# simzero/cudaParticlesFoam

Hardware: AMD Instinct MI355X
Metric: Mparticle-steps/s (higher is better)
Workload: dtype f64

## Files before the change

cudaparticlesfoam_amd/csrc/cpf_api.cpp:

```cpp
#include <hip/hip_runtime.h>

#include <algorithm>
#include <cmath>
#include <cstring>
#include <condition_variable>
#include <mutex>
#include <string>
#include <thread>
#include <utility>
#include <vector>

#include "cpf.h"
#include "cpf_device.h"
#include "cpf_internal.h"
#include "cpf_walk.h"

struct cpf_context {
    int device = 0;
    hipStream_t ownStream = nullptr, stream = nullptr;
    mutable std::string err;
    bool haveMesh = false, haveU = false;
    cpf::HostTables host;
    int32_t* d_cellOff = nullptr;
    double4* d_planes = nullptr;
    int32_t* d_nbr = nullptr;
    int32_t *d_groupOff = nullptr, *d_groupNbr = nullptr;
    bool zFold = true;
    double4* d_U = nullptr;
    double* d_U3 = nullptr;
    double* d_boxRec = nullptr;
    bool boxRecords = true;
    double4* d_cellRec = nullptr;
    unsigned long long* d_occupied = nullptr;
    hipEvent_t evFieldFlag = nullptr;
    bool fieldFlagPending = false;
    unsigned long long* h_occupied = nullptr;
    int64_t nSecondRecords = 0;
    float* d_cellBox = nullptr;
    int32_t* d_curveRank = nullptr;
    int sortMethod = 2;
    int sortCurve = -1;
    int32_t* d_binOff = nullptr;
    int32_t* d_binCells = nullptr;
    size_t meshBytes = 0;
    int64_t cap = 0, n = 0;
    double *x = nullptr, *y = nullptr, *z = nullptr, *vel = nullptr;
    int32_t* cell = nullptr;
    int64_t* gid = nullptr;
    double *x2 = nullptr, *y2 = nullptr, *z2 = nullptr;
    int32_t* cell2 = nullptr;
    int64_t* gid2 = nullptr;
    bool located = false;
    void* scratch = nullptr;
    size_t scratchBytes = 0;
    unsigned long long* d_counters = nullptr;
    uint32_t seed = 1591593751u;
    uint32_t stepCounter = 0;
    int sortInterval = 50;
    uint32_t lastSortStep = 0;
    bool stats = false;
    int stepVariant = -1;
    bool vtuBinary = false;
    bool mixedRecords = true;
    double nonplanarTol = cpf::kNonPlanarTolDefault;
    bool splitNonplanar = true;
    cpf_mesh_quality quality{};
    int64_t nParent = 0;
    std::vector<int32_t> first;
    int32_t* d_parentOf = nullptr;
    double* d_Uparent = nullptr;
    cpf::StreamState streamState;
    int64_t lastStepN = -1;
    int lastStepCycles = 1;
    bool zSettled = false;
    bool lastStepZSettled = false;
    double* d_tetPos = nullptr; int32_t* d_tets = nullptr; double* d_vertVel = nullptr;
    int64_t nTetVerts = 0, nTets = 0; int tetsPerCell = 0; bool haveVertVel = false;
    double* d_vertCone = nullptr;
    double* d_vertApex = nullptr;
    bool vertexFast = true;
    std::string vertConeWhy;
    std::thread writer;
    bool writerLive = false;
    int writerStatus = CPF_OK;
    void* snapDev = nullptr; void* snapHost = nullptr;
    size_t snapBytes = 0;
    hipStream_t ioStream = nullptr;
    hipEvent_t evSnap = nullptr, evCopied = nullptr;
    double frameKE = 0.0;
    std::mutex keMutex; std::condition_variable keCv; bool keReady = false;
    int timingStride = 1;
    uint64_t timingLaunch = 0;
    bool timing = false;
    std::vector<std::pair<hipEvent_t, hipEvent_t>> events;
    std::vector<hipEvent_t> eventPool;
};

namespace {

std::string g_createError = "";
std::mutex g_mutex;

struct WriterRegistry {
    std::vector<cpf_context*> live;
    ~WriterRegistry();
} g_writers;

int fail(const cpf_context* ctx, int code, const std::string& msg) {
    if (ctx) ctx->err = msg;
    else { std::lock_guard<std::mutex> lk(g_mutex); g_createError = msg; }
    return code;
}

#define CPF_HIP(ctx, call)                                                                              \
    do {                                                                                                \
        hipError_t e__ = (call);                                                                        \
        if (e__ != hipSuccess)                                                                          \
            return fail(ctx, CPF_ERR_HIP, std::string(#call) + ": " + hipGetErrorString(e__));          \
    } while (0)

#define CPF_REQUIRE(ctx, cond, code, msg) \
    do { if (!(cond)) return fail(ctx, code, msg); } while (0)

template <typename T>
void freeDev(T*& p) { if (p) { (void)hipFree(p); p = nullptr; } }

cpf::MeshView meshView(const cpf_context* c) {
    cpf::MeshView m;
    m.cellOff = c->d_cellOff; m.planes = c->d_planes; m.nbr = c->d_nbr; m.U = c->d_U;
    m.groupOff = c->d_groupOff; m.groupNbr = c->d_groupNbr;
    m.cellRec = c->d_cellRec;
    m.boxRec = c->boxRecords ? reinterpret_cast<const double4*>(c->d_boxRec) : nullptr;
    m.nCells = (int32_t)c->host.nCells;
    m.allHex = (c->host.minCellFaces == 6 && c->host.maxCellFaces == 6 && c->host.nGroups() == 0) ? 1 : 0;
    m.zPairLast = c->host.zPairLast ? 1 : 0;
    m.zThin = (c->host.zThin && c->zFold) ? 1 : 0;
    m.zSide0 = c->host.zSide0 ? 1 : 0;
    m.mixed = (c->d_cellRec && !m.allHex) ? (c->host.nBigCells > 0 ? 2 : 1) : 0;
    return m;
}
cpf::GridView gridView(const cpf_context* c) {
    cpf::GridView g;
    for (int k = 0; k < 3; ++k) {
        g.origin[k] = c->host.origin[k]; g.invBin[k] = c->host.invBin[k];
        g.lo[k] = c->host.lo[k]; g.hi[k] = c->host.hi[k]; g.dims[k] = c->host.dims[k];
    }
    g.binOff = c->d_binOff; g.binCells = c->d_binCells;
    return g;
}

int ensureScratch(cpf_context* ctx, size_t bytes) {
    if (bytes <= ctx->scratchBytes) return CPF_OK;
    CPF_HIP(ctx, hipStreamSynchronize(ctx->stream));
    freeDev(ctx->scratch);
    ctx->scratchBytes = 0;
    CPF_HIP(ctx, hipMalloc(&ctx->scratch, bytes));
    ctx->scratchBytes = bytes;
    return CPF_OK;
}

int sortEndBit(const cpf_context* ctx) {
    int bits = 1;
    while (((int64_t)1 << bits) < ctx->host.nCells + 2) ++bits;
    return std::min(bits + ctx->host.subBits[0] + ctx->host.subBits[1] + ctx->host.subBits[2], 32);
}

void freeMesh(cpf_context* c) {
    freeDev(c->d_cellOff); freeDev(c->d_planes); freeDev(c->d_nbr); freeDev(c->d_groupOff); freeDev(c->d_groupNbr); freeDev(c->d_U); freeDev(c->d_U3); freeDev(c->d_cellRec); freeDev(c->d_boxRec); freeDev(c->d_cellBox); freeDev(c->d_curveRank);
    freeDev(c->d_binOff); freeDev(c->d_binCells);
    c->haveMesh = c->haveU = false; c->meshBytes = 0;
    c->nSecondRecords = 0;
    freeDev(c->d_parentOf); freeDev(c->d_Uparent);
    c->first.clear(); c->nParent = 0; c->quality = cpf_mesh_quality{};
    freeDev(c->d_tetPos); freeDev(c->d_tets); freeDev(c->d_vertVel);
    c->haveVertVel = false; c->nTets = c->nTetVerts = 0; c->tetsPerCell = 0;
}
void freeCloud(cpf_context* c) {
    freeDev(c->x); freeDev(c->y); freeDev(c->z); freeDev(c->vel); freeDev(c->cell); freeDev(c->gid);
    freeDev(c->x2); freeDev(c->y2); freeDev(c->z2); freeDev(c->cell2); freeDev(c->gid2);
    c->cap = c->n = 0; c->located = false; c->zSettled = false;
}

cpf_mesh_quality toQuality(const cpf::MeshQuality& q, int64_t nDerived) {
    cpf_mesh_quality r{};
    r.maxNonPlanarity = q.maxEta; r.worstFace = q.worstFace;
    r.maxNonConvexity = q.maxXi; r.worstCell = q.worstCell;
    r.nCells = q.nCells; r.nFlaggedCells = q.nFlagged; r.nBadCells = q.nBad; r.nDerivedCells = nDerived;
    r.tol = q.tol;
    return r;
}

template <typename Label>
int setMeshImpl(cpf_context* ctx, const double* points, int64_t nPoints, const Label* faceOffsets,
                const Label* faceVerts, int64_t nFaces, const Label* owner, const Label* neighbour,
                int64_t nInternal, int64_t nCells) {
    CPF_REQUIRE(ctx, ctx, CPF_ERR_ARG, "null context");
    CPF_REQUIRE(ctx, points && faceOffsets && faceVerts && owner && (neighbour || nInternal == 0), CPF_ERR_ARG,
                "cpf_set_mesh: null array");
    cpf::MeshQuality q;
    std::string why = cpf::measure_mesh<Label>(points, nPoints, faceOffsets, faceVerts, nFaces, owner, neighbour, nInternal,
                                               nCells, ctx->nonplanarTol, q);
    if (!why.empty()) return fail(ctx, CPF_ERR_MESH, "cpf_set_mesh: " + why);
    bool derive = ctx->splitNonplanar && q.decompose();
    cpf::DerivedMesh dm;
    cpf::HostTables t;
    if (derive) {
        why = cpf::derive_mesh<Label>(points, nPoints, faceOffsets, faceVerts, nFaces, owner, neighbour, nInternal, nCells, q, dm);
        if (why.empty())
            why = cpf::build_tables<int64_t>(dm.points.data(), dm.nPoints, dm.faceOff.data(), dm.faceVerts.data(), dm.nFaces,
                                             dm.owner.data(), dm.neighbour.data(), dm.nInternal, dm.nCells, t);
        for (int64_t c = 0; c < nCells && why.empty() && derive; ++c)
            if (dm.first[(size_t)c + 1] - dm.first[(size_t)c] == 1) {
                const int32_t d = dm.first[(size_t)c];
                if (t.cellOff[(size_t)d + 1] - t.cellOff[(size_t)d] > q.cellOff[(size_t)c + 1] - q.cellOff[(size_t)c]) derive = false;
            }
    }
    if (!derive) {
        why = cpf::build_tables<Label>(points, nPoints, faceOffsets, faceVerts, nFaces, owner, neighbour, nInternal, nCells, t);
    }
    if (!why.empty()) return fail(ctx, CPF_ERR_MESH, "cpf_set_mesh: " + why);
    CPF_HIP(ctx, hipSetDevice(ctx->device));
    CPF_HIP(ctx, hipStreamSynchronize(ctx->stream));
    freeMesh(ctx);
    ctx->streamState.flatField = false;
    ctx->host = std::move(t);
    ctx->nParent = nCells;
    ctx->quality = toQuality(q, ctx->host.nCells);
    nCells = ctx->host.nCells;
    const cpf::HostTables& h = ctx->host;
    auto up = [&](auto*& dptr, const void* src, size_t bytes) -> hipError_t {
        hipError_t e = hipMalloc((void**)&dptr, std::max<size_t>(bytes, 16));
        if (e != hipSuccess) return e;
        ctx->meshBytes += bytes;
        return hipMemcpy(dptr, src, bytes, hipMemcpyHostToDevice);
    };
    CPF_HIP(ctx, up(ctx->d_cellOff, h.cellOff.data(), h.cellOff.size() * 4));
    CPF_HIP(ctx, up(ctx->d_planes, h.planes.data(), h.planes.size() * 8));
    CPF_HIP(ctx, up(ctx->d_nbr, h.nbr.data(), h.nbr.size() * 4));
    CPF_HIP(ctx, up(ctx->d_groupOff, h.groupOff.data(), h.groupOff.size() * 4));
    CPF_HIP(ctx, up(ctx->d_groupNbr, h.groupNbr.data(), h.groupNbr.size() * 4));
    CPF_HIP(ctx, up(ctx->d_binOff, h.binOff.data(), h.binOff.size() * 4));
    CPF_HIP(ctx, up(ctx->d_binCells, h.binCells.data(), h.binCells.size() * 4));
    CPF_HIP(ctx, up(ctx->d_cellBox, h.cellBox.data(), h.cellBox.size() * 4));
    CPF_HIP(ctx, up(ctx->d_curveRank, h.curveRank.data(), h.curveRank.size() * 4));
    if (derive) {
        ctx->first = std::move(dm.first);
        CPF_HIP(ctx, up(ctx->d_parentOf, dm.parent.data(), dm.parent.size() * 4));
        CPF_HIP(ctx, hipMalloc((void**)&ctx->d_Uparent, (size_t)ctx->nParent * 3 * sizeof(double)));
        ctx->meshBytes += (size_t)ctx->nParent * 24;
    }
    CPF_HIP(ctx, hipMalloc((void**)&ctx->d_U, (size_t)nCells * sizeof(double4)));
    CPF_HIP(ctx, hipMalloc((void**)&ctx->d_U3, (size_t)nCells * 3 * sizeof(double)));
    CPF_HIP(ctx, hipMemset(ctx->d_U, 0, (size_t)nCells * sizeof(double4)));
    if (ctx->host.minCellFaces == 6 && ctx->host.maxCellFaces == 6 && ctx->host.nGroups() == 0) {
        CPF_HIP(ctx, hipMalloc((void**)&ctx->d_cellRec, (size_t)nCells * 8 * sizeof(double4)));
        CPF_HIP(ctx, cpf::launch_build_cell_records(ctx->stream, ctx->d_planes, ctx->d_nbr, ctx->d_U, ctx->d_cellRec, nCells));
        CPF_HIP(ctx, hipStreamSynchronize(ctx->stream));
        ctx->meshBytes += (size_t)nCells * 256;
        if (!h.boxRec.empty()) CPF_HIP(ctx, up(ctx->d_boxRec, h.boxRec.data(), h.boxRec.size() * 8));
    } else if (ctx->host.nHugeCells * 4 <= nCells && ctx->mixedRecords) {
        std::vector<int32_t> recB((size_t)nCells, -1);
        int64_t nSecond = 0;
        for (int64_t c = 0; c < nCells; ++c) {
            const int nf = ctx->host.cellOff[(size_t)c + 1] - ctx->host.cellOff[(size_t)c];
            if (nf > 6 && nf <= 12) recB[(size_t)c] = (int32_t)(nCells + nSecond++);
        }
        CPF_REQUIRE(ctx, nCells + nSecond < ((int64_t)1 << 31), CPF_ERR_MESH, "cpf_set_mesh: too many cell records");
        int32_t* d_recB = nullptr;
        hipError_t e = hipSuccess;
        if (nSecond > 0) e = up(d_recB, recB.data(), recB.size() * 4);
        if (e == hipSuccess) e = hipMalloc((void**)&ctx->d_cellRec, (size_t)(nCells + nSecond) * 8 * sizeof(double4));
        if (e == hipSuccess) e = cpf::launch_build_cell_records_mixed(ctx->stream, ctx->d_cellOff, ctx->d_planes, ctx->d_nbr, ctx->d_U, d_recB,
                                                                      ctx->d_cellRec, nCells);
        if (e == hipSuccess) e = hipStreamSynchronize(ctx->stream);
        freeDev(d_recB);
        CPF_HIP(ctx, e);
        ctx->nSecondRecords = nSecond;
        ctx->meshBytes += (size_t)(nCells + nSecond) * 256;
        if (!h.boxRec.empty() && nSecond == 0) CPF_HIP(ctx, up(ctx->d_boxRec, h.boxRec.data(), h.boxRec.size() * 8));
    }
    ctx->meshBytes += (size_t)nCells * (sizeof(double4) + 24);
    ctx->haveMesh = true;
    ctx->located = false;
    ctx->zSettled = false;
    if (ctx->h_occupied) ctx->h_occupied[0] = ctx->h_occupied[1] = 0;
    return CPF_OK;
}

}

namespace {
WriterRegistry::~WriterRegistry() {
    for (cpf_context* c : live)
        if (c->writerLive && c->writer.joinable()) { c->writer.join(); c->writerLive = false; }
}
}

namespace cpf {
bool vtu_binary(const cpf_context* ctx) { return ctx && ctx->vtuBinary; }
bool context_derived(const cpf_context* ctx) { return ctx && ctx->d_parentOf != nullptr; }
void* context_stream(const cpf_context* ctx) { return (void*)ctx->stream; }
int context_device(const cpf_context* ctx) { return ctx->device; }
bool context_timing(const cpf_context* ctx) { return ctx->timing; }
int64_t context_cells(const cpf_context* ctx) { return ctx->haveMesh ? ctx->host.nCells : 0; }
bool context_step_settled_z(const cpf_context* ctx) { return ctx->lastStepZSettled; }
}

namespace {
std::string tetFanDefect(const double* pos, const int32_t* tets, int64_t nCells, int tetsPerCell) {
    auto P = [&](int32_t v, int k) { return pos[3 * (int64_t)v + k]; };
    const double fourPi = 12.566370614359172;
    std::vector<uint64_t> edges;
    for (int64_t c = 0; c < nCells; ++c) {
        const int32_t* t0 = tets + 4 * c * tetsPerCell;
        const int32_t apex = t0[0];
        double omega = 0.0;
        int sign = 0;
        for (int k = 0; k < tetsPerCell; ++k) {
            const int32_t* ix = t0 + 4 * k;
            if (ix[0] != apex) return "cell " + std::to_string(c) + ": its tets do not share their first vertex";
            double e[3][3], len[3];
            for (int j = 0; j < 3; ++j) {
                for (int q = 0; q < 3; ++q) e[j][q] = P(ix[j + 1], q) - P(apex, q);
                len[j] = std::sqrt(e[j][0] * e[j][0] + e[j][1] * e[j][1] + e[j][2] * e[j][2]);
            }
            const double det = e[0][0] * (e[1][1] * e[2][2] - e[1][2] * e[2][1]) - e[0][1] * (e[1][0] * e[2][2] - e[1][2] * e[2][0]) +
                               e[0][2] * (e[1][0] * e[2][1] - e[1][1] * e[2][0]);
            const double scale = len[0] * len[1] * len[2];
            if (!(std::fabs(det) * 1e5 > scale)) return "cell " + std::to_string(c) + ": a flat (or badly conditioned) tet";
            const int sg = det > 0 ? 1 : -1;
            if (sign == 0) sign = sg;
            else if (sg != sign) return "cell " + std::to_string(c) + ": tets of both orientations";
            auto dot = [&](int i, int j) { return e[i][0] * e[j][0] + e[i][1] * e[j][1] + e[i][2] * e[j][2]; };
            omega += 2.0 * std::atan2(std::fabs(det), scale + dot(0, 1) * len[2] + dot(0, 2) * len[1] + dot(1, 2) * len[0]);
        }
        if (std::fabs(omega - fourPi) > 1e-6) return "cell " + std::to_string(c) + ": the tets' solid angles at the apex do not add up to 4 pi";
        edges.clear();
        for (int k = 0; k < tetsPerCell; ++k) {
            const int32_t* ix = t0 + 4 * k;
            for (int j = 0; j < 3; ++j) edges.push_back(((uint64_t)(uint32_t)ix[1 + j] << 32) | (uint32_t)ix[1 + (j + 1) % 3]);
        }
        std::sort(edges.begin(), edges.end());
        for (size_t i = 0; i < edges.size(); ++i) {
            const uint64_t rev = (edges[i] << 32) | (edges[i] >> 32);
            if ((i > 0 && edges[i] == edges[i - 1]) || !std::binary_search(edges.begin(), edges.end(), rev))
                return "cell " + std::to_string(c) + ": the tets' base triangles do not form a closed surface";
        }
    }
    return "";
}

hipError_t layOutField(cpf_context* ctx, const double* dU3, int64_t nCells) {
    const bool ask = ctx->host.zSide0 && ctx->d_occupied && ctx->h_occupied;
    ctx->streamState.flatField = false;
    ctx->fieldFlagPending = false;
    hipError_t e = hipSuccess;
    if (ask) e = hipMemsetAsync(ctx->d_occupied + 2, 0, 8, ctx->stream);
    if (e == hipSuccess) e = cpf::launch_u3_to_u4(ctx->stream, dU3, ctx->d_U, nCells, ask ? ctx->d_occupied + 2 : nullptr);
    if (e == hipSuccess && ctx->d_cellRec) e = cpf::launch_update_record_velocity(ctx->stream, ctx->d_U, ctx->d_cellRec, ctx->d_boxRec, nCells);
    if (e == hipSuccess && ask) {
        e = hipMemcpyAsync(ctx->h_occupied + 2, ctx->d_occupied + 2, 8, hipMemcpyDeviceToHost, ctx->stream);
        if (e == hipSuccess) e = hipEventRecord(ctx->evFieldFlag, ctx->stream);
        ctx->fieldFlagPending = e == hipSuccess;
    }
    return e;
}
std::string resolveSubCells(const cpf_context* ctx, int64_t n, const double* xyz, const int32_t* cell, std::vector<int32_t>& out) {
    const cpf::HostTables& h = ctx->host;
    out.resize((size_t)n);
    for (int64_t i = 0; i < n; ++i) {
        const int32_t c = cell[i];
        if (c < 0) { out[(size_t)i] = c; continue; }
        if (c >= ctx->nParent) return "cell[" + std::to_string(i) + "] = " + std::to_string(c) + " is not a cell of the mesh";
        const double px = xyz[3 * i], py = xyz[3 * i + 1], pz = xyz[3 * i + 2];
        int32_t pick = ctx->first[(size_t)c];
        double pickWorst = HUGE_VAL;
        for (int32_t d = ctx->first[(size_t)c]; d < ctx->first[(size_t)c + 1]; ++d) {
            double worst = -HUGE_VAL;
            for (int32_t s = h.cellOff[(size_t)d]; s < h.cellOff[(size_t)d + 1]; ++s) {
                const double* pl = &h.planes[4 * (size_t)s];
                worst = std::max(worst, std::fma(-pl[2], pz, std::fma(-pl[1], py, std::fma(-pl[0], px, pl[3]))));
            }
            if (worst < cpf::kTol) { pick = d; break; }
            if (worst < pickWorst) { pickWorst = worst; pick = d; }
        }
        out[(size_t)i] = pick;
    }
    return std::string();
}
void fieldFlagArrived(cpf_context* ctx) {
    if (!ctx->fieldFlagPending) return;
    ctx->streamState.flatField = ctx->h_occupied[2] == 0;
    ctx->fieldFlagPending = false;
}
void pollFieldFlag(cpf_context* ctx) {
    if (ctx->fieldFlagPending && hipEventQuery(ctx->evFieldFlag) == hipSuccess) fieldFlagArrived(ctx);
}
}

extern "C" {

int cpf_abi_version(void) { return CPF_ABI_VERSION; }

int cpf_create(int device, cpf_context** out) {
    if (!out) return fail(nullptr, CPF_ERR_ARG, "cpf_create: out is null");
    *out = nullptr;
    int count = 0;
    hipError_t e = hipGetDeviceCount(&count);
    if (e != hipSuccess || count <= 0)
        return fail(nullptr, CPF_ERR_HIP,
                    std::string("cpf_create: no HIP device available (") + hipGetErrorString(e) + ")");
    if (device < 0 || device >= count) return fail(nullptr, CPF_ERR_ARG, "cpf_create: device index out of range");
    e = hipSetDevice(device);
    if (e != hipSuccess) return fail(nullptr, CPF_ERR_HIP, std::string("hipSetDevice: ") + hipGetErrorString(e));
    cpf_context* ctx = new (std::nothrow) cpf_context();
    if (!ctx) return fail(nullptr, CPF_ERR_NOMEM, "cpf_create: out of host memory");
    ctx->device = device;
    e = hipStreamCreateWithFlags(&ctx->ownStream, hipStreamNonBlocking);
    if (e == hipSuccess) e = hipMalloc((void**)&ctx->d_counters, (cpf::kCounterSlots * 4 + 4) * sizeof(unsigned long long));
    if (e == hipSuccess) e = hipMemset(ctx->d_counters, 0, (cpf::kCounterSlots * 4 + 4) * sizeof(unsigned long long));
    if (e == hipSuccess) e = hipMalloc((void**)&ctx->d_occupied, 32);
    if (e == hipSuccess) e = hipHostMalloc((void**)&ctx->h_occupied, 32, hipHostMallocDefault);
    if (e == hipSuccess) { ctx->h_occupied[0] = ctx->h_occupied[1] = 0; ctx->h_occupied[2] = 1; ctx->streamState.occupiedHost = ctx->h_occupied; }
    if (e == hipSuccess) e = hipEventCreateWithFlags(&ctx->evFieldFlag, hipEventDisableTiming);
    if (e == hipSuccess) e = hipMalloc((void**)&ctx->streamState.d_grab, cpf::kStreamGrabBytes);
    if (e == hipSuccess) e = hipMemset(ctx->streamState.d_grab, 0, cpf::kStreamGrabBytes);
    if (e == hipSuccess) {
        int cus = 0;
        e = hipDeviceGetAttribute(&cus, hipDeviceAttributeMultiprocessorCount, device);
        if (e == hipSuccess && cus > 0) ctx->streamState.numCU = cus;
    }
    if (e == hipSuccess) {
        ctx->streamState.hitSpillWaves = 32 * ctx->streamState.numCU;
        e = hipMalloc((void**)&ctx->streamState.d_hitSpill,
                      (size_t)ctx->streamState.hitSpillWaves * cpf::kStreamHitSpillDoubles * sizeof(double));
    }
    if (e != hipSuccess) {
        std::string m = std::string("cpf_create: ") + hipGetErrorString(e);
        if (ctx->ownStream) (void)hipStreamDestroy(ctx->ownStream);
        delete ctx;
        return fail(nullptr, CPF_ERR_HIP, m);
    }
    ctx->stream = ctx->ownStream;
    *out = ctx;
    return CPF_OK;
}

int cpf_destroy(cpf_context* ctx) {
    if (!ctx) return CPF_OK;
    (void)cpf_write_vtu_wait(ctx);
    (void)hipSetDevice(ctx->device);
    (void)hipStreamSynchronize(ctx->stream);
    freeMesh(ctx); freeCloud(ctx);
    freeDev(ctx->scratch); freeDev(ctx->d_counters); freeDev(ctx->streamState.d_grab); freeDev(ctx->streamState.d_hitSpill);
    freeDev(ctx->d_occupied);
    if (ctx->evFieldFlag) { (void)hipEventDestroy(ctx->evFieldFlag); ctx->evFieldFlag = nullptr; }
    if (ctx->h_occupied) { (void)hipHostFree(ctx->h_occupied); ctx->h_occupied = nullptr; ctx->streamState.occupiedHost = nullptr; }
    freeDev(ctx->d_tetPos); freeDev(ctx->d_tets); freeDev(ctx->d_vertVel); freeDev(ctx->d_vertCone); freeDev(ctx->d_vertApex);
    freeDev(ctx->snapDev);
    if (ctx->snapHost) { (void)hipHostFree(ctx->snapHost); ctx->snapHost = nullptr; }
    if (ctx->evSnap) (void)hipEventDestroy(ctx->evSnap);
    if (ctx->evCopied) (void)hipEventDestroy(ctx->evCopied);
    if (ctx->ioStream) (void)hipStreamDestroy(ctx->ioStream);
    for (auto& p : ctx->events) { (void)hipEventDestroy(p.first); (void)hipEventDestroy(p.second); }
    for (auto& ev : ctx->eventPool) (void)hipEventDestroy(ev);
    if (ctx->ownStream) (void)hipStreamDestroy(ctx->ownStream);
    delete ctx;
    return CPF_OK;
}

const char* cpf_last_error(const cpf_context* ctx) {
    if (ctx) return ctx->err.c_str();
    std::lock_guard<std::mutex> lk(g_mutex);
    return g_createError.c_str();
}

int cpf_set_stream(cpf_context* ctx, void* hip_stream) {
    CPF_REQUIRE(ctx, ctx, CPF_ERR_ARG, "null context");
    CPF_HIP(ctx, hipStreamSynchronize(ctx->stream));
    fieldFlagArrived(ctx);
    ctx->stream = (hipStream_t)hip_stream;
    return CPF_OK;
}

int cpf_use_own_stream(cpf_context* ctx) {
    CPF_REQUIRE(ctx, ctx, CPF_ERR_ARG, "null context");
    CPF_HIP(ctx, hipStreamSynchronize(ctx->stream));
    fieldFlagArrived(ctx);
    ctx->stream = ctx->ownStream;
    return CPF_OK;
}

int cpf_synchronize(cpf_context* ctx) {
    CPF_REQUIRE(ctx, ctx, CPF_ERR_ARG, "null context");
    CPF_HIP(ctx, hipStreamSynchronize(ctx->stream));
    return CPF_OK;
}

int cpf_set_mesh(cpf_context* ctx, const double* points, int64_t nPoints, const int32_t* faceOffsets,
                 const int32_t* faceVerts, int64_t nFaces, const int32_t* owner, const int32_t* neighbour,
                 int64_t nInternal, int64_t nCells) {
    return setMeshImpl<int32_t>(ctx, points, nPoints, faceOffsets, faceVerts, nFaces, owner, neighbour, nInternal,
                                nCells);
}
int cpf_set_mesh_l64(cpf_context* ctx, const double* points, int64_t nPoints, const int64_t* faceOffsets,
                     const int64_t* faceVerts, int64_t nFaces, const int64_t* owner, const int64_t* neighbour,
                     int64_t nInternal, int64_t nCells) {
    return setMeshImpl<int64_t>(ctx, points, nPoints, faceOffsets, faceVerts, nFaces, owner, neighbour, nInternal,
                                nCells);
}

int cpf_build_mesh_tables_host(const double* points, int64_t nPoints, const int32_t* faceOffsets, const int32_t* faceVerts,
                               int64_t nFaces, const int32_t* owner, const int32_t* neighbour, int64_t nInternal, int64_t nCells,
                               int64_t* nSlots, int64_t* nGroups, int64_t* nMembers, int32_t* cellOff, double* planes,
                               int32_t* nbr, int32_t* groupOff, int32_t* groupNbr) {
    if (!points || !faceOffsets || !faceVerts || !owner || (!neighbour && nInternal != 0)) return CPF_ERR_ARG;
    cpf::HostTables t;
    try {
        const std::string why = cpf::build_tables<int32_t>(points, nPoints, faceOffsets, faceVerts, nFaces, owner, neighbour, nInternal, nCells, t);
        if (!why.empty()) return CPF_ERR_MESH;
    } catch (const std::bad_alloc&) {
        return CPF_ERR_NOMEM;
    }
    const int64_t g = t.nGroups(), mem = t.groupOff[(size_t)g];
    if (nSlots) *nSlots = t.nSlots;
    if (nGroups) *nGroups = g;
    if (nMembers) *nMembers = mem;
    if (cellOff) std::memcpy(cellOff, t.cellOff.data(), t.cellOff.size() * 4);
    if (planes) std::memcpy(planes, t.planes.data(), t.planes.size() * 8);
    if (nbr) std::memcpy(nbr, t.nbr.data(), t.nbr.size() * 4);
    if (groupOff) std::memcpy(groupOff, t.groupOff.data(), (size_t)(g + 1) * 4);
    if (groupNbr) std::memcpy(groupNbr, t.groupNbr.data(), (size_t)mem * 4);
    return CPF_OK;
}

int cpf_mesh_flags_host(const double* points, int64_t nPoints, const int32_t* faceOffsets, const int32_t* faceVerts,
                        int64_t nFaces, const int32_t* owner, const int32_t* neighbour, int64_t nInternal, int64_t nCells,
                        int32_t* allHex, int32_t* zLayered, int32_t* zThin, int32_t* mixed) {
    if (!points || !faceOffsets || !faceVerts || !owner || (!neighbour && nInternal != 0)) return CPF_ERR_ARG;
    cpf::HostTables t;
    try {
        const std::string why = cpf::build_tables<int32_t>(points, nPoints, faceOffsets, faceVerts, nFaces, owner, neighbour, nInternal, nCells, t);
        if (!why.empty()) return CPF_ERR_MESH;
    } catch (const std::bad_alloc&) {
        return CPF_ERR_NOMEM;
    }
    const bool hex = t.minCellFaces == 6 && t.maxCellFaces == 6 && t.nGroups() == 0;
    if (allHex) *allHex = hex ? 1 : 0;
    if (zLayered) *zLayered = t.zPairLast ? 1 : 0;
    if (zThin) *zThin = t.zThin ? 1 : 0;
    if (mixed) *mixed = hex ? 0 : (t.nHugeCells * 4 <= nCells ? (t.nBigCells > 0 ? 2 : 1) : 0);
    return CPF_OK;
}

int cpf_mesh_box_records_host(const double* points, int64_t nPoints, const int32_t* faceOffsets, const int32_t* faceVerts,
                              int64_t nFaces, const int32_t* owner, const int32_t* neighbour, int64_t nInternal, int64_t nCells,
                              int32_t* isBox, double* boxRec) {
    if (!points || !faceOffsets || !faceVerts || !owner || (!neighbour && nInternal != 0)) return CPF_ERR_ARG;
    cpf::HostTables t;
    try {
        const std::string why = cpf::build_tables<int32_t>(points, nPoints, faceOffsets, faceVerts, nFaces, owner, neighbour, nInternal, nCells, t);
        if (!why.empty()) return CPF_ERR_MESH;
    } catch (const std::bad_alloc&) {
        return CPF_ERR_NOMEM;
    }
    if (isBox) *isBox = t.boxRec.empty() ? 0 : 1;
    if (boxRec && !t.boxRec.empty()) std::memcpy(boxRec, t.boxRec.data(), t.boxRec.size() * 8);
    return CPF_OK;
}

int cpf_mesh_quality_host(const double* points, int64_t nPoints, const int32_t* faceOffsets, const int32_t* faceVerts,
                          int64_t nFaces, const int32_t* owner, const int32_t* neighbour, int64_t nInternal, int64_t nCells,
                          double tol, int split, cpf_mesh_quality* out) {
    if (!points || !faceOffsets || !faceVerts || !owner || (!neighbour && nInternal != 0) || !out || !(tol > 0.0)) return CPF_ERR_ARG;
    try {
        cpf::MeshQuality q;
        if (!cpf::measure_mesh<int32_t>(points, nPoints, faceOffsets, faceVerts, nFaces, owner, neighbour, nInternal, nCells, tol, q).empty())
            return CPF_ERR_MESH;
        int64_t nDerived = nCells;
        if (split && q.decompose()) {
            cpf::DerivedMesh dm;
            if (!cpf::derive_mesh<int32_t>(points, nPoints, faceOffsets, faceVerts, nFaces, owner, neighbour, nInternal, nCells, q, dm).empty())
                return CPF_ERR_MESH;
            nDerived = dm.nCells;
        }
        *out = toQuality(q, nDerived);
    } catch (const std::bad_alloc&) {
        return CPF_ERR_NOMEM;
    }
    return CPF_OK;
}

int cpf_build_derived_mesh_host(const double* points, int64_t nPoints, const int32_t* faceOffsets, const int32_t* faceVerts,
                                int64_t nFaces, const int32_t* owner, const int32_t* neighbour, int64_t nInternal, int64_t nCells,
                                double tol, int64_t sizes[5], double* pointsOut, int32_t* faceOffOut, int32_t* faceVertsOut,
                                int32_t* ownerOut, int32_t* neighbourOut, int32_t* first) {
    if (!points || !faceOffsets || !faceVerts || !owner || (!neighbour && nInternal != 0) || !sizes || !(tol > 0.0)) return CPF_ERR_ARG;
    try {
        cpf::MeshQuality q;
        if (!cpf::measure_mesh<int32_t>(points, nPoints, faceOffsets, faceVerts, nFaces, owner, neighbour, nInternal, nCells, tol, q).empty())
            return CPF_ERR_MESH;
        cpf::DerivedMesh dm;
        if (!cpf::derive_mesh<int32_t>(points, nPoints, faceOffsets, faceVerts, nFaces, owner, neighbour, nInternal, nCells, q, dm).empty())
            return CPF_ERR_MESH;
        if (dm.faceVerts.size() > (size_t)INT32_MAX) return CPF_ERR_MESH;
        sizes[0] = dm.nPoints; sizes[1] = dm.nFaces; sizes[2] = (int64_t)dm.faceVerts.size(); sizes[3] = dm.nInternal; sizes[4] = dm.nCells;
        auto narrow = [](const std::vector<int64_t>& v, int32_t* o) { if (o) for (size_t i = 0; i < v.size(); ++i) o[i] = (int32_t)v[i]; };
        if (pointsOut) std::memcpy(pointsOut, dm.points.data(), dm.points.size() * 8);
        narrow(dm.faceOff, faceOffOut); narrow(dm.faceVerts, faceVertsOut); narrow(dm.owner, ownerOut); narrow(dm.neighbour, neighbourOut);
        if (first) std::memcpy(first, dm.first.data(), dm.first.size() * 4);
    } catch (const std::bad_alloc&) {
        return CPF_ERR_NOMEM;
    }
    return CPF_OK;
}

int cpf_get_mesh_quality(const cpf_context* ctx, cpf_mesh_quality* out) {
    CPF_REQUIRE(ctx, ctx && out, CPF_ERR_ARG, "null argument");
    CPF_REQUIRE(ctx, ctx->haveMesh, CPF_ERR_STATE, "cpf_get_mesh_quality: call cpf_set_mesh first");
    *out = ctx->quality;
    return CPF_OK;
}

int cpf_cells_to_parent_dev(cpf_context* ctx, const int32_t* in, int32_t* out, int64_t n) {
    CPF_REQUIRE(ctx, ctx, CPF_ERR_ARG, "null context");
    CPF_REQUIRE(ctx, ctx->haveMesh, CPF_ERR_STATE, "cpf_cells_to_parent_dev: call cpf_set_mesh first");
    CPF_REQUIRE(ctx, n >= 0 && (n == 0 || (in && out)), CPF_ERR_ARG, "cpf_cells_to_parent_dev: bad arguments");
    CPF_HIP(ctx, hipSetDevice(ctx->device));
    if (ctx->d_parentOf) CPF_HIP(ctx, cpf::launch_cells_to_parent(ctx->stream, in, out, ctx->d_parentOf, n, ctx->host.nCells));
    else if (n > 0 && in != out) CPF_HIP(ctx, hipMemcpyAsync(out, in, (size_t)n * 4, hipMemcpyDeviceToDevice, ctx->stream));
    return CPF_OK;
}

int cpf_mesh_info(const cpf_context* ctx, int64_t* nCells, int64_t* nSlots, int64_t* deviceBytes) {
    CPF_REQUIRE(ctx, ctx, CPF_ERR_ARG, "null context");
    CPF_REQUIRE(ctx, ctx->haveMesh, CPF_ERR_STATE, "cpf_mesh_info: no mesh set");
    if (nCells) *nCells = ctx->host.nCells;
    if (nSlots) *nSlots = ctx->host.nSlots;
    if (deviceBytes) *deviceBytes = (int64_t)ctx->meshBytes;
    return CPF_OK;
}

int cpf_get_mesh_tables(const cpf_context* ctx, int32_t* cellOff, double* planes, int32_t* nbr) {
    CPF_REQUIRE(ctx, ctx, CPF_ERR_ARG, "null context");
    CPF_REQUIRE(ctx, ctx->haveMesh, CPF_ERR_STATE, "cpf_get_mesh_tables: no mesh set");
    const cpf::HostTables& h = ctx->host;
    if (cellOff) std::memcpy(cellOff, h.cellOff.data(), h.cellOff.size() * 4);
    if (planes) std::memcpy(planes, h.planes.data(), h.planes.size() * 8);
    if (nbr) std::memcpy(nbr, h.nbr.data(), h.nbr.size() * 4);
    return CPF_OK;
}

int cpf_get_mesh_groups(const cpf_context* ctx, int64_t* nGroups, int64_t* nMembers, int32_t* groupOff, int32_t* groupNbr) {
    CPF_REQUIRE(ctx, ctx, CPF_ERR_ARG, "null context");
    CPF_REQUIRE(ctx, ctx->haveMesh, CPF_ERR_STATE, "cpf_get_mesh_groups: no mesh set");
    const cpf::HostTables& h = ctx->host;
    const int64_t g = h.nGroups();
    if (nGroups) *nGroups = g;
    if (nMembers) *nMembers = h.groupOff[(size_t)g];
    if (groupOff) std::memcpy(groupOff, h.groupOff.data(), (size_t)(g + 1) * 4);
    if (groupNbr) std::memcpy(groupNbr, h.groupNbr.data(), (size_t)h.groupOff[(size_t)g] * 4);
    return CPF_OK;
}

int cpf_get_mesh_flags(const cpf_context* ctx, int32_t* allHex, int32_t* zLayered, int32_t* zThin, int32_t* mixed) {
    CPF_REQUIRE(ctx, ctx, CPF_ERR_ARG, "null context");
    CPF_REQUIRE(ctx, ctx->haveMesh, CPF_ERR_STATE, "cpf_get_mesh_flags: no mesh set");
    const cpf::MeshView m = meshView(ctx);
    if (allHex) *allHex = m.allHex;
    if (zLayered) *zLayered = m.zPairLast;
    if (zThin) *zThin = m.zThin;
    if (mixed) *mixed = m.mixed;
    return CPF_OK;
}

int cpf_set_velocity(cpf_context* ctx, const double* U, int64_t nCells) {
    CPF_REQUIRE(ctx, ctx, CPF_ERR_ARG, "null context");
    CPF_REQUIRE(ctx, ctx->haveMesh, CPF_ERR_STATE, "cpf_set_velocity: call cpf_set_mesh first");
    CPF_REQUIRE(ctx, U && nCells == ctx->nParent, CPF_ERR_ARG, "cpf_set_velocity: U is null or nCells differs from the mesh");
    CPF_HIP(ctx, hipSetDevice(ctx->device));
    if (ctx->d_parentOf) {
        CPF_HIP(ctx, hipMemcpyAsync(ctx->d_Uparent, U, (size_t)nCells * 24, hipMemcpyHostToDevice, ctx->stream));
        CPF_HIP(ctx, cpf::launch_gather_parent_u3(ctx->stream, ctx->d_Uparent, ctx->d_parentOf, ctx->d_U3, ctx->host.nCells));
    } else {
        CPF_HIP(ctx, hipMemcpyAsync(ctx->d_U3, U, (size_t)nCells * 24, hipMemcpyHostToDevice, ctx->stream));
    }
    CPF_HIP(ctx, layOutField(ctx, ctx->d_U3, ctx->host.nCells));
    CPF_HIP(ctx, hipStreamSynchronize(ctx->stream));
    fieldFlagArrived(ctx);
    ctx->haveU = true;
    return CPF_OK;
}

int cpf_set_velocity_dev(cpf_context* ctx, const double* dU, int64_t nCells) {
    CPF_REQUIRE(ctx, ctx, CPF_ERR_ARG, "null context");
    CPF_REQUIRE(ctx, ctx->haveMesh, CPF_ERR_STATE, "cpf_set_velocity_dev: call cpf_set_mesh first");
    CPF_REQUIRE(ctx, dU && nCells == ctx->nParent, CPF_ERR_ARG, "cpf_set_velocity_dev: bad arguments");
    CPF_HIP(ctx, hipSetDevice(ctx->device));
    if (ctx->d_parentOf) {
        CPF_HIP(ctx, cpf::launch_gather_parent_u3(ctx->stream, dU, ctx->d_parentOf, ctx->d_U3, ctx->host.nCells));
        dU = ctx->d_U3;
    }
    CPF_HIP(ctx, layOutField(ctx, dU, ctx->host.nCells));
    ctx->haveU = true;
    return CPF_OK;
}

int cpf_alloc_particles(cpf_context* ctx, int64_t capacity) {
    CPF_REQUIRE(ctx, ctx, CPF_ERR_ARG, "null context");
    CPF_REQUIRE(ctx, capacity > 0 && capacity < ((int64_t)1 << 31), CPF_ERR_ARG, "cpf_alloc_particles: capacity must be in (0, 2^31)");
    CPF_HIP(ctx, hipSetDevice(ctx->device));
    CPF_HIP(ctx, hipStreamSynchronize(ctx->stream));
    freeCloud(ctx);
    const size_t c = (size_t)capacity;
    CPF_HIP(ctx, hipMalloc((void**)&ctx->x, c * 8));
    CPF_HIP(ctx, hipMalloc((void**)&ctx->y, c * 8));
    CPF_HIP(ctx, hipMalloc((void**)&ctx->z, c * 8));
    CPF_HIP(ctx, hipMalloc((void**)&ctx->vel, c * 24));
    CPF_HIP(ctx, hipMalloc((void**)&ctx->cell, c * 4));
    CPF_HIP(ctx, hipMalloc((void**)&ctx->gid, c * 8));
    CPF_HIP(ctx, hipMemsetAsync(ctx->vel, 0, c * 24, ctx->stream));
    CPF_HIP(ctx, hipMemsetAsync(ctx->cell, 0xFF, c * 4, ctx->stream));
    ctx->cap = capacity;
    return CPF_OK;
}

int cpf_seed_box(cpf_context* ctx, int64_t n, const double lower[3], const double upper[3], int order) {
    CPF_REQUIRE(ctx, ctx, CPF_ERR_ARG, "null context");
    CPF_REQUIRE(ctx, lower && upper && n > 0, CPF_ERR_ARG, "cpf_seed_box: bad arguments");
    if (ctx->cap < n) { int r = cpf_alloc_particles(ctx, n); if (r) return r; }
    CPF_HIP(ctx, hipSetDevice(ctx->device));
    CPF_HIP(ctx, cpf::launch_seed_box(ctx->stream, ctx->x, ctx->y, ctx->z, 0, n, lower, upper, order));
    CPF_HIP(ctx, cpf::launch_iota64(ctx->stream, ctx->gid, n, 0));
    CPF_HIP(ctx, hipMemsetAsync(ctx->cell, 0xFF, (size_t)n * 4, ctx->stream));
    ctx->n = n; ctx->located = false; ctx->zSettled = false;
    return CPF_OK;
}

int cpf_set_particles(cpf_context* ctx, int64_t n, const double* xyz, const int32_t* cell) {
    CPF_REQUIRE(ctx, ctx, CPF_ERR_ARG, "null context");
    CPF_REQUIRE(ctx, xyz && n > 0, CPF_ERR_ARG, "cpf_set_particles: bad arguments");
    if (ctx->cap < n) { int r = cpf_alloc_particles(ctx, n); if (r) return r; }
    CPF_HIP(ctx, hipSetDevice(ctx->device));
    ctx->zSettled = false;
    int r = ensureScratch(ctx, (size_t)n * 24);
    if (r) return r;
    CPF_HIP(ctx, hipMemcpyAsync(ctx->scratch, xyz, (size_t)n * 24, hipMemcpyHostToDevice, ctx->stream));
    CPF_HIP(ctx, cpf::launch_unpack_xyz(ctx->stream, (const double*)ctx->scratch, ctx->x, ctx->y, ctx->z, n));
    CPF_HIP(ctx, cpf::launch_iota64(ctx->stream, ctx->gid, n, 0));
    std::vector<int32_t> sub;
    if (cell && ctx->d_parentOf) {
        std::string why = resolveSubCells(ctx, n, xyz, cell, sub);
        if (!why.empty()) { (void)hipStreamSynchronize(ctx->stream); return fail(ctx, CPF_ERR_ARG, "cpf_set_particles: " + why); }
        cell = sub.data();
    }
    if (cell) CPF_HIP(ctx, hipMemcpyAsync(ctx->cell, cell, (size_t)n * 4, hipMemcpyHostToDevice, ctx->stream));
    else CPF_HIP(ctx, hipMemsetAsync(ctx->cell, 0xFF, (size_t)n * 4, ctx->stream));
    CPF_HIP(ctx, hipStreamSynchronize(ctx->stream));
    ctx->n = n; ctx->located = cell != nullptr;
    return CPF_OK;
}

int cpf_locate_initial_dev(cpf_context* ctx, const double* x, const double* y, const double* z, int32_t* cell,
                           int64_t n) {
    CPF_REQUIRE(ctx, ctx, CPF_ERR_ARG, "null context");
    CPF_REQUIRE(ctx, ctx->haveMesh, CPF_ERR_STATE, "cpf_locate_initial: call cpf_set_mesh first");
    CPF_REQUIRE(ctx, n >= 0 && (n == 0 || (x && y && z && cell)), CPF_ERR_ARG, "cpf_locate_initial: null array");
    CPF_HIP(ctx, hipSetDevice(ctx->device));
    CPF_HIP(ctx, cpf::launch_locate_initial(ctx->stream, x, y, z, cell, n, meshView(ctx), gridView(ctx)));
    return CPF_OK;
}

int cpf_locate_initial(cpf_context* ctx, int64_t* nOutside) {
    CPF_REQUIRE(ctx, ctx, CPF_ERR_ARG, "null context");
    CPF_REQUIRE(ctx, ctx->n > 0, CPF_ERR_STATE, "cpf_locate_initial: no particles (seed or set them first)");
    ctx->zSettled = false;
    int r = cpf_locate_initial_dev(ctx, ctx->x, ctx->y, ctx->z, ctx->cell, ctx->n);
    if (r) return r;
    ctx->located = true;
    if (nOutside) {
        unsigned long long* cnt = ctx->d_counters + cpf::kCounterSlots * 4;
        CPF_HIP(ctx, hipMemsetAsync(cnt, 0, 8, ctx->stream));
        CPF_HIP(ctx, cpf::launch_count_negative(ctx->stream, ctx->cell, ctx->n, cnt));
        unsigned long long h = 0;
        CPF_HIP(ctx, hipMemcpyAsync(&h, cnt, 8, hipMemcpyDeviceToHost, ctx->stream));
        CPF_HIP(ctx, hipStreamSynchronize(ctx->stream));
        *nOutside = (int64_t)h;
    }
    return CPF_OK;
}

static cpf::VertexField vertexField(const cpf_context* ctx) {
    return {ctx->d_tetPos, ctx->d_tets, ctx->d_vertVel, ctx->tetsPerCell, ctx->vertexFast ? ctx->d_vertCone : nullptr,
            reinterpret_cast<const double4*>(ctx->d_vertApex)};
}

#ifndef CPF_TIMING_EVENT_FLAGS
#define CPF_TIMING_EVENT_FLAGS hipEventReleaseToDevice
#endif

int cpf_step_dev(cpf_context* ctx, double* x, double* y, double* z, int32_t* cell, const int64_t* gid, double* vel,
                 int64_t n, double dt, double D, uint32_t step0, int nCycles, unsigned flags) {
    CPF_REQUIRE(ctx, ctx, CPF_ERR_ARG, "null context");
    CPF_REQUIRE(ctx, ctx->haveMesh, CPF_ERR_STATE, "cpf_step: call cpf_set_mesh first");
    CPF_REQUIRE(ctx, ctx->haveU, CPF_ERR_STATE, "cpf_step: call cpf_set_velocity first");
    CPF_REQUIRE(ctx, n >= 0 && nCycles >= 0, CPF_ERR_ARG, "cpf_step: negative count");
    CPF_REQUIRE(ctx, n == 0 || (x && y && z && cell), CPF_ERR_ARG, "cpf_step: null particle array");
    CPF_REQUIRE(ctx, std::isfinite(dt) && std::isfinite(D) && D >= 0.0, CPF_ERR_ARG, "cpf_step: dt/D not finite or D < 0");
    CPF_REQUIRE(ctx, !(flags & CPF_STEP_STORE_VEL) || vel, CPF_ERR_ARG, "cpf_step: CPF_STEP_STORE_VEL needs a vel array");
    CPF_HIP(ctx, hipSetDevice(ctx->device));
    const bool vertexU = (flags & CPF_STEP_VERTEX_VELOCITY) != 0;
    CPF_REQUIRE(ctx, !vertexU || (ctx->haveVertVel && ctx->nTets == (int64_t)ctx->tetsPerCell * ctx->host.nCells), CPF_ERR_STATE,
                "cpf_step: CPF_STEP_VERTEX_VELOCITY needs cpf_set_tets and cpf_set_vertex_velocity for the current mesh");
    const cpf::MeshView m = meshView(ctx);
    const cpf::VertexField vf = vertexField(ctx);
    const bool fuse = (flags & CPF_STEP_FUSE_CYCLES) != 0;
    pollFieldFlag(ctx);
    bool settled = (flags & CPF_STEP_Z_SETTLED) != 0;
    ctx->lastStepZSettled = false;
    const int nLaunch = fuse ? 1 : nCycles;
    const int cycPerLaunch = fuse ? nCycles : 1;
    for (int c = 0; c < nLaunch; ++c) {
        const cpf::StepPlan plan = cpf::plan_step(m, ctx->streamState, ctx->stepVariant, vertexU ? &vf : nullptr, n, cycPerLaunch, D,
                                                  flags, ctx->stats);
        hipEvent_t e0 = nullptr, e1 = nullptr;
        const bool timed = ctx->timing && (ctx->timingLaunch++ % (uint64_t)ctx->timingStride) == 0;
        const bool stamped = timed && n > 0 && plan.stamped();
        if (timed) {
            auto take = [&](hipEvent_t& ev) -> hipError_t {
                if (!ctx->eventPool.empty()) { ev = ctx->eventPool.back(); ctx->eventPool.pop_back(); return hipSuccess; }
                return hipEventCreateWithFlags(&ev, CPF_TIMING_EVENT_FLAGS);
            };
            CPF_HIP(ctx, take(e0)); CPF_HIP(ctx, take(e1));
            if (!stamped) CPF_HIP(ctx, hipEventRecord(e0, ctx->stream));
        }
        ctx->lastStepN = n; ctx->lastStepCycles = cycPerLaunch;
        const hipError_t le = cpf::launch_step(plan, ctx->stream, x, y, z, cell, gid, vel, n, dt, D, step0 + (uint32_t)c, cycPerLaunch,
                                               ctx->seed, m, ctx->stats ? ctx->d_counters : nullptr, vertexU ? &vf : nullptr,
                                               ctx->streamState, settled, stamped ? e0 : nullptr, stamped ? e1 : nullptr);
        if (le != hipSuccess) {
            if (e0) ctx->eventPool.push_back(e0);
            if (e1) ctx->eventPool.push_back(e1);
        }
        CPF_HIP(ctx, le);
        if (n > 0 && cycPerLaunch > 0) settled = plan.flat();
        if (timed) {
            if (!stamped) CPF_HIP(ctx, hipEventRecord(e1, ctx->stream));
            ctx->events.emplace_back(e0, e1);
        }
    }
    ctx->lastStepZSettled = settled;
    return CPF_OK;
}

int cpf_step(cpf_context* ctx, double dt, double D, int nCycles, unsigned flags) {
    CPF_REQUIRE(ctx, ctx, CPF_ERR_ARG, "null context");
    CPF_REQUIRE(ctx, ctx->n > 0, CPF_ERR_STATE, "cpf_step: no particles");
    CPF_REQUIRE(ctx, ctx->located, CPF_ERR_STATE, "cpf_step: particles have no cells yet (call cpf_locate_initial)");
    if ((flags & CPF_STEP_STORE_VEL) && ctx->vel) {
        CPF_HIP(ctx, hipSetDevice(ctx->device));
        CPF_HIP(ctx, hipMemsetAsync(ctx->vel, 0, (size_t)ctx->n * 24, ctx->stream));
    }
    const bool settled = ctx->zSettled;
    ctx->zSettled = false;
    int r = cpf_step_dev(ctx, ctx->x, ctx->y, ctx->z, ctx->cell, ctx->gid, ctx->vel, ctx->n, dt, D, ctx->stepCounter,
                         nCycles, (flags & ~CPF_STEP_Z_SETTLED) | (settled ? CPF_STEP_Z_SETTLED : 0u));
    if (r != CPF_OK) return r;
    ctx->zSettled = ctx->lastStepZSettled;
    if (!(dt == 0.0 && D == 0.0)) ctx->stepCounter += (uint32_t)nCycles;
    if (ctx->sortInterval > 0 && ctx->stepCounter - ctx->lastSortStep >= (uint32_t)ctx->sortInterval) {
        r = cpf_sort_by_cell(ctx);
        ctx->lastSortStep = ctx->stepCounter;
    }
    return r;
}

int cpf_seed_box_dev(cpf_context* ctx, double* x, double* y, double* z, int64_t first, int64_t n,
                     const double lower[3], const double upper[3], int order) {
    CPF_REQUIRE(ctx, ctx, CPF_ERR_ARG, "null context");
    CPF_REQUIRE(ctx, n >= 0 && first >= 0 && lower && upper && (n == 0 || (x && y && z)), CPF_ERR_ARG, "cpf_seed_box_dev: bad arguments");
    CPF_HIP(ctx, hipSetDevice(ctx->device));
    CPF_HIP(ctx, cpf::launch_seed_box(ctx->stream, x, y, z, first, n, lower, upper, order));
    return CPF_OK;
}

namespace {
int sortImpl(cpf_context* ctx, double* x, double* y, double* z, int32_t* cell, int64_t* gid, int64_t n, double* ox, double* oy,
             double* oz, int32_t* ocell, int64_t* ogid, double* vel3) {
    CPF_REQUIRE(ctx, ctx->haveMesh, CPF_ERR_STATE, "cpf_sort_by_cell: call cpf_set_mesh first");
    CPF_REQUIRE(ctx, n >= 0 && n < ((int64_t)1 << 31) && (n == 0 || (x && y && z && cell)), CPF_ERR_ARG, "cpf_sort_by_cell: bad arguments");
    CPF_REQUIRE(ctx, ctx->host.nCells < ((int64_t)1 << 26) - 2, CPF_ERR_STATE, "cpf_sort_by_cell: more than 2^26 cells");
    CPF_HIP(ctx, hipSetDevice(ctx->device));
    const int endBit = sortEndBit(ctx);
    const bool census = ctx->streamState.densityLookup != 0 && ctx->d_occupied && ctx->h_occupied;
    const bool curve = ctx->d_curveRank != nullptr && (ctx->sortCurve == 1 || (ctx->sortCurve < 0 && n < 8 * ctx->host.nCells));
    int r = ensureScratch(ctx, cpf::sort_scratch_bytes(n, endBit));
    if (r) return r;
    CPF_HIP(ctx, cpf::sort_by_cell(ctx->stream, x, y, z, cell, gid, vel3, n, endBit, ctx->d_cellBox, ctx->host.subBits,
                                   ctx->host.subOrder, ctx->scratch, ctx->scratchBytes, ox, oy, oz, ocell, ogid, census ? ctx->d_occupied : nullptr,
                                   curve ? ctx->d_curveRank : nullptr, ctx->sortMethod));
    if (census)
        CPF_HIP(ctx, hipMemcpyAsync(ctx->h_occupied, ctx->d_occupied, 16, hipMemcpyDeviceToHost, ctx->stream));
    return CPF_OK;
}
}

int cpf_sort_by_cell_dev(cpf_context* ctx, double* x, double* y, double* z, int32_t* cell, int64_t* gid, int64_t n) {
    CPF_REQUIRE(ctx, ctx, CPF_ERR_ARG, "null context");
    if (n <= 1) return CPF_OK;
    return sortImpl(ctx, x, y, z, cell, gid, n, nullptr, nullptr, nullptr, nullptr, nullptr, nullptr);
}

int cpf_sort_by_cell_dev_to(cpf_context* ctx, const double* x, const double* y, const double* z, const int32_t* cell,
                            const int64_t* gid, double* ox, double* oy, double* oz, int32_t* ocell, int64_t* ogid, int64_t n) {
    CPF_REQUIRE(ctx, ctx, CPF_ERR_ARG, "null context");
    CPF_REQUIRE(ctx, n == 0 || (ox && oy && oz && ocell && (ogid || !gid)), CPF_ERR_ARG, "cpf_sort_by_cell_dev_to: null output array");
    CPF_REQUIRE(ctx, n == 0 || (ox != x && oy != y && oz != z && ocell != cell), CPF_ERR_ARG, "cpf_sort_by_cell_dev_to: outputs alias inputs");
    if (n <= 0) return CPF_OK;
    if (n == 1) {
        CPF_HIP(ctx, hipSetDevice(ctx->device));
        CPF_HIP(ctx, hipMemcpyAsync(ox, x, 8, hipMemcpyDeviceToDevice, ctx->stream));
        CPF_HIP(ctx, hipMemcpyAsync(oy, y, 8, hipMemcpyDeviceToDevice, ctx->stream));
        CPF_HIP(ctx, hipMemcpyAsync(oz, z, 8, hipMemcpyDeviceToDevice, ctx->stream));
        CPF_HIP(ctx, hipMemcpyAsync(ocell, cell, 4, hipMemcpyDeviceToDevice, ctx->stream));
        if (gid) CPF_HIP(ctx, hipMemcpyAsync(ogid, gid, 8, hipMemcpyDeviceToDevice, ctx->stream));
        return CPF_OK;
    }
    return sortImpl(ctx, const_cast<double*>(x), const_cast<double*>(y), const_cast<double*>(z), const_cast<int32_t*>(cell),
                    const_cast<int64_t*>(gid), n, ox, oy, oz, ocell, ogid, nullptr);
}

int cpf_sort_by_cell(cpf_context* ctx) {
    CPF_REQUIRE(ctx, ctx, CPF_ERR_ARG, "null context");
    CPF_REQUIRE(ctx, ctx->n > 0 && ctx->located, CPF_ERR_STATE, "cpf_sort_by_cell: no located particles");
    if (ctx->n <= 1) return CPF_OK;
    if (ctx->x2 == nullptr) {
        CPF_HIP(ctx, hipSetDevice(ctx->device));
        const size_t c = (size_t)ctx->cap;
        void* b[5] = {nullptr, nullptr, nullptr, nullptr, nullptr};
        const size_t bytes[5] = {c * 8, c * 8, c * 8, c * 4, c * 8};
        hipError_t e = hipSuccess;
        for (int k = 0; k < 5 && e == hipSuccess; ++k) e = hipMalloc(&b[k], bytes[k]);
        if (e == hipSuccess) e = hipMemsetAsync(b[3], 0xFF, bytes[3], ctx->stream);
        if (e != hipSuccess) {
            for (int k = 0; k < 5; ++k) if (b[k]) (void)hipFree(b[k]);
            CPF_HIP(ctx, e);
        }
        ctx->x2 = (double*)b[0]; ctx->y2 = (double*)b[1]; ctx->z2 = (double*)b[2];
        ctx->cell2 = (int32_t*)b[3]; ctx->gid2 = (int64_t*)b[4];
    }
    int r = sortImpl(ctx, ctx->x, ctx->y, ctx->z, ctx->cell, ctx->gid, ctx->n, ctx->x2, ctx->y2, ctx->z2, ctx->cell2, ctx->gid2,
                     ctx->vel);
    if (r) return r;
    std::swap(ctx->x, ctx->x2); std::swap(ctx->y, ctx->y2); std::swap(ctx->z, ctx->z2);
    std::swap(ctx->cell, ctx->cell2); std::swap(ctx->gid, ctx->gid2);
    return CPF_OK;
}

int cpf_num_particles(const cpf_context* ctx, int64_t* n) {
    CPF_REQUIRE(ctx, ctx && n, CPF_ERR_ARG, "null argument");
    *n = ctx->n;
    return CPF_OK;
}

int cpf_get_particles(cpf_context* ctx, double* xyzw, int32_t* cell, double* vel) {
    CPF_REQUIRE(ctx, ctx, CPF_ERR_ARG, "null context");
    CPF_REQUIRE(ctx, ctx->n > 0, CPF_ERR_STATE, "cpf_get_particles: no particles");
    CPF_HIP(ctx, hipSetDevice(ctx->device));
    const size_t n = (size_t)ctx->n;
    auto al = [](size_t b) { return (b + 255) & ~(size_t)255; };
    int r = ensureScratch(ctx, al(n * 32) + al(n * 4) + al(n * 32));
    if (r) return r;
    char* p = (char*)ctx->scratch;
    double* dX = (double*)p; p += al(n * 32);
    int32_t* dC = (int32_t*)p; p += al(n * 4);
    double* dV = (double*)p;
    CPF_HIP(ctx, cpf::launch_pack_by_gid(ctx->stream, ctx->x, ctx->y, ctx->z, ctx->cell, ctx->gid, ctx->vel,
                                         xyzw ? dX : nullptr, cell ? dC : nullptr, vel ? dV : nullptr, ctx->n));
    if (cell && ctx->d_parentOf) CPF_HIP(ctx, cpf::launch_cells_to_parent(ctx->stream, dC, dC, ctx->d_parentOf, ctx->n, ctx->host.nCells));
    if (xyzw) CPF_HIP(ctx, hipMemcpyAsync(xyzw, dX, n * 32, hipMemcpyDeviceToHost, ctx->stream));
    if (cell) CPF_HIP(ctx, hipMemcpyAsync(cell, dC, n * 4, hipMemcpyDeviceToHost, ctx->stream));
    if (vel) CPF_HIP(ctx, hipMemcpyAsync(vel, dV, n * 32, hipMemcpyDeviceToHost, ctx->stream));
    CPF_HIP(ctx, hipStreamSynchronize(ctx->stream));
    return CPF_OK;
}

int cpf_get_counters(cpf_context* ctx, int64_t out[4]) {
    CPF_REQUIRE(ctx, ctx && out, CPF_ERR_ARG, "null argument");
    CPF_HIP(ctx, hipSetDevice(ctx->device));
    std::vector<unsigned long long> h((size_t)cpf::kCounterSlots * 4);
    CPF_HIP(ctx, hipMemcpyAsync(h.data(), ctx->d_counters, h.size() * 8, hipMemcpyDeviceToHost, ctx->stream));
    CPF_HIP(ctx, hipStreamSynchronize(ctx->stream));
    for (int k = 0; k < 4; ++k) {
        unsigned long long sum = 0;
        for (int s = 0; s < cpf::kCounterSlots; ++s) sum += h[(size_t)s * 4 + k];
        out[k] = (int64_t)sum;
    }
    return CPF_OK;
}

int cpf_set_option(cpf_context* ctx, const char* key, double value) {
    CPF_REQUIRE(ctx, ctx && key, CPF_ERR_ARG, "null argument");
    const std::string k(key);
    if (k == "step_variant") {
        CPF_REQUIRE(ctx, value >= -1 && value <= 5 && value == (int)value, CPF_ERR_ARG, "step_variant must be -1..5");
#ifndef CPF_EXPERIMENTS
        CPF_REQUIRE(ctx, value != 1 && value != 2 && value != 5, CPF_ERR_ARG,
                    "step_variant 1, 2 and 5 are experiments (measured slower on every mesh) and not in this build: make EXPERIMENTS=1");
#endif
        ctx->stepVariant = (int)value;
        return CPF_OK;
    }
    if (k == "vertex_fast") {
        CPF_REQUIRE(ctx, value == 0 || value == 1, CPF_ERR_ARG, "vertex_fast must be 0 or 1");
        ctx->vertexFast = value != 0;
        return CPF_OK;
    }
    if (k == "z_fold") {
        CPF_REQUIRE(ctx, value == 0 || value == 1, CPF_ERR_ARG, "z_fold must be 0 or 1");
        ctx->zFold = value != 0;
        return CPF_OK;
    }
    if (k == "mixed_records") {
        CPF_REQUIRE(ctx, value == 0 || value == 1, CPF_ERR_ARG, "mixed_records must be 0 or 1");
        ctx->mixedRecords = value != 0;
        return CPF_OK;
    }
    if (k == "flat_walk") {
        CPF_REQUIRE(ctx, value == 0 || value == 1, CPF_ERR_ARG, "flat_walk must be 0 or 1");
        ctx->streamState.flat = (int)value;
        return CPF_OK;
    }
    if (k == "flat_z") {
        CPF_REQUIRE(ctx, value == 0 || value == 1, CPF_ERR_ARG, "flat_z must be 0 or 1");
        ctx->streamState.flatZ = (int)value;
        return CPF_OK;
    }
    if (k == "box_records") {
        CPF_REQUIRE(ctx, value == 0 || value == 1, CPF_ERR_ARG, "box_records must be 0 or 1");
        ctx->boxRecords = value != 0;
        return CPF_OK;
    }
    if (k == "stream_tiles_per_chunk") {
        CPF_REQUIRE(ctx, value >= 1 && value <= 1024 && value == (int)value, CPF_ERR_ARG, "stream_tiles_per_chunk must be 1..1024");
        ctx->streamState.tilesPerChunk = (int)value;
        return CPF_OK;
    }
    if (k == "sort_key_bits") {
        CPF_REQUIRE(ctx, ctx->haveMesh, CPF_ERR_STATE, "sort_key_bits: call cpf_set_mesh first");
        const int v = (int)value, nb[3] = {v / 100, (v / 10) % 10, v % 10};
        CPF_REQUIRE(ctx, value == v && v >= 0 && nb[0] <= 9 && nb[0] + nb[1] + nb[2] <= 12, CPF_ERR_ARG, "sort_key_bits: at most 12 bits");
        for (int a = 0; a < 3; ++a) {
            const float f = std::ldexp(1.0f, nb[a] - ctx->host.subBits[a]);
            for (size_t c = 0; c < ctx->host.cellBox.size() / 6; ++c) ctx->host.cellBox[6 * c + 3 + a] *= f;
            ctx->host.subBits[a] = nb[a];
        }
        CPF_HIP(ctx, hipSetDevice(ctx->device));
        CPF_HIP(ctx, hipMemcpyAsync(ctx->d_cellBox, ctx->host.cellBox.data(), ctx->host.cellBox.size() * 4, hipMemcpyHostToDevice, ctx->stream));
        CPF_HIP(ctx, hipStreamSynchronize(ctx->stream));
        return CPF_OK;
    }
    if (k == "stream_tail_fraction") {
        CPF_REQUIRE(ctx, value >= 0 && value <= 1, CPF_ERR_ARG, "stream_tail_fraction must be in [0, 1]");
        ctx->streamState.tailFraction = value;
        return CPF_OK;
    }
    if (k == "coop_max_cells") {
        CPF_REQUIRE(ctx, value >= 0 && value <= (1 << 24), CPF_ERR_ARG, "coop_max_cells must be in [0, 2^24]");
        ctx->streamState.coopMaxCells = (int)value;
        return CPF_OK;
    }
    if (k == "stream_lookup") {
        CPF_REQUIRE(ctx, value == -1 || (value >= 0 && value <= 6 && value == (int)value), CPF_ERR_ARG, "stream_lookup must be -1 (auto) or 0 ... 6");
        ctx->streamState.lookup = (int)value;
        return CPF_OK;
    }
    if (k == "stream_lookup_by_density") {
        CPF_REQUIRE(ctx, value == 0 || value == 1, CPF_ERR_ARG, "stream_lookup_by_density must be 0 or 1");
        ctx->streamState.densityLookup = (int)value;
        return CPF_OK;
    }
    if (k == "sort_method") {
        CPF_REQUIRE(ctx, value == 0 || value == 2, CPF_ERR_ARG, "sort_method must be 2 (this library's radix sort) or 0 (hipcub's)");
        ctx->sortMethod = (int)value;
        return CPF_OK;
    }
    if (k == "sort_curve") {
        CPF_REQUIRE(ctx, value == -1 || value == 0 || value == 1, CPF_ERR_ARG, "sort_curve must be -1 (by regime), 0 (cell id) or 1 (Morton rank)");
        ctx->sortCurve = (int)value;
        return CPF_OK;
    }
    if (k == "vtu_binary") {
        CPF_REQUIRE(ctx, value == 0 || value == 1, CPF_ERR_ARG, "vtu_binary must be 0 or 1");
        ctx->vtuBinary = value != 0;
        return CPF_OK;
    }
    if (k == "stream_debug") {
        ctx->streamState.debug = (int)value;
        return CPF_OK;
    }
    if (k == "stream_waves_per_cu") {
        CPF_REQUIRE(ctx, value >= 0 && value <= 32 && value == (int)value, CPF_ERR_ARG, "stream_waves_per_cu must be 0..32 (0 = auto)");
        ctx->streamState.wavesPerCU = (int)value;
        return CPF_OK;
    }
    if (k == "sort_interval") {
        CPF_REQUIRE(ctx, value >= 0 && value <= 1e9, CPF_ERR_ARG, "sort_interval must be >= 0 (0 = never)");
        ctx->sortInterval = (int)value;
        return CPF_OK;
    }
    if (k == "timing_stride") {
        CPF_REQUIRE(ctx, value >= 1 && value <= 1e6 && value == (int)value, CPF_ERR_ARG, "timing_stride must be an integer >= 1");
        ctx->timingStride = (int)value;
        return CPF_OK;
    }
    if (k == "stats") {
        ctx->stats = value != 0;
        return CPF_OK;
    }
    if (k == "nonplanar_tol") {
        CPF_REQUIRE(ctx, value > 0.0 && std::isfinite(value), CPF_ERR_ARG, "nonplanar_tol must be a positive number");
        ctx->nonplanarTol = value;
        return CPF_OK;
    }
    if (k == "split_nonplanar") {
        CPF_REQUIRE(ctx, value == 0 || value == 1, CPF_ERR_ARG, "split_nonplanar must be 0 or 1");
        ctx->splitNonplanar = value != 0;
        return CPF_OK;
    }
    return fail(ctx, CPF_ERR_ARG, "cpf_set_option: unknown key '" + k + "'");
}

}
namespace cpf {
void set_context_error(cpf_context* ctx, const char* message) {
    if (ctx) ctx->err = message ? message : "";
}
}
extern "C" {

int cpf_step_kernel_name(cpf_context* ctx, double D, unsigned flags, char* buf, size_t bufBytes) {
    CPF_REQUIRE(ctx, ctx && buf && bufBytes > 0, CPF_ERR_ARG, "null argument");
    CPF_REQUIRE(ctx, ctx->haveMesh, CPF_ERR_STATE, "cpf_step_kernel_name: call cpf_set_mesh first");
    const cpf::MeshView m = meshView(ctx);
    const cpf::VertexField vf = vertexField(ctx);
    pollFieldFlag(ctx);
    const bool vertexU = (flags & CPF_STEP_VERTEX_VELOCITY) != 0;
    const int64_t n = (vertexU ? ctx->lastStepN > 0 : ctx->lastStepN >= 0) ? ctx->lastStepN : ctx->n;
    const cpf::StepPlan p = cpf::plan_step(m, ctx->streamState, ctx->stepVariant, vertexU ? &vf : nullptr, n,
                                           (flags & CPF_STEP_FUSE_CYCLES) ? ctx->lastStepCycles : 1, D, flags, ctx->stats);
    const char* b[2] = {"false", "true"};
    char tmp[192];
    if (p.kernel == cpf::StepPlan::kStreamVertex)
        snprintf(tmp, sizeof tmp, "cpf::step_kernel_stream_vertex<%s, %s, %s, %s, %d> (cone locate)", b[p.brown], b[p.reflect],
                 b[p.storeVel], b[p.stats], p.lookup);
    else if (p.kernel == cpf::StepPlan::kVertex)
        snprintf(tmp, sizeof tmp, "cpf::step_kernel_vertex<%s, %s, %s> (%s)", b[p.brown], b[p.reflect], b[p.storeVel],
                 p.cone ? "cone locate" : (ctx->d_vertCone || ctx->vertConeWhy.empty() ? "all tets" : ("all tets: " + ctx->vertConeWhy).c_str()));
    else if (p.kernel == cpf::StepPlan::kAhead)
        snprintf(tmp, sizeof tmp, "cpf::step_kernel_ahead<%s, %s>", b[p.reflect], b[p.stats]);
    else if (p.kernel == cpf::StepPlan::kStream)
        snprintf(tmp, sizeof tmp, "cpf::step_kernel_stream<%s, %s, %s, %s, %d>", b[p.brown], b[p.reflect], b[p.storeVel], b[p.stats], p.lookup);
    else if (p.kernel == cpf::StepPlan::kCoop)
        snprintf(tmp, sizeof tmp, "cpf::step_kernel_coop<%s, %s, %s, %s>", b[p.brown], b[p.reflect], b[p.storeVel], b[p.stats]);
    else snprintf(tmp, sizeof tmp, "cpf::step_kernel<%d, %s, %s, %s>", (int)p.kernel, b[p.brown], b[p.reflect], b[p.storeVel]);
    snprintf(buf, bufBytes, "%s", tmp);
    return CPF_OK;
}

int cpf_set_seed(cpf_context* ctx, uint32_t seed) {
    CPF_REQUIRE(ctx, ctx, CPF_ERR_ARG, "null context");
    ctx->seed = seed;
    return CPF_OK;
}

int cpf_pack_leavers_dev(cpf_context* ctx, double* x, double* y, double* z, int32_t* cell, int64_t* gid, int64_t n,
                         const int32_t* cellLo_dev, int nRanks, int myRank, double* sendbuf, int64_t sendCapacity,
                         int64_t* counts_dev, int64_t* nStay_dev) {
    CPF_REQUIRE(ctx, ctx, CPF_ERR_ARG, "null context");
    CPF_REQUIRE(ctx, n >= 0 && n < ((int64_t)1 << 31) && nRanks >= 1 && nRanks <= CPF_MAX_RANKS && myRank >= 0 && myRank < nRanks,
                CPF_ERR_ARG, "cpf_pack_leavers_dev: bad sizes (1 .. CPF_MAX_RANKS ranks)");
    CPF_REQUIRE(ctx, cellLo_dev && counts_dev && nStay_dev && (sendbuf || sendCapacity == 0) && (n == 0 || (x && y && z && cell)),
                CPF_ERR_ARG, "cpf_pack_leavers_dev: null array");
    CPF_REQUIRE(ctx, !ctx->d_parentOf, CPF_ERR_MESH, "cpf_pack_leavers_dev: the mesh has cells decomposed into tets "
                "(cpf_get_mesh_quality): ownership ranges are parent ids, the cloud's cells derived ids");
    CPF_HIP(ctx, hipSetDevice(ctx->device));
    int r = ensureScratch(ctx, cpf::handoff_scratch_bytes(n, nRanks));
    if (r) return r;
    CPF_HIP(ctx, cpf::pack_leavers(ctx->stream, x, y, z, cell, gid, n, cellLo_dev, nRanks, myRank, sendbuf,
                                   sendCapacity, counts_dev, nStay_dev, ctx->scratch, ctx->scratchBytes));
    return CPF_OK;
}

int cpf_cell_histogram_dev(cpf_context* ctx, const int32_t* cell, int64_t n, double scale, double* weights_dev) {
    CPF_REQUIRE(ctx, ctx, CPF_ERR_ARG, "null context");
    CPF_REQUIRE(ctx, ctx->haveMesh, CPF_ERR_STATE, "cpf_cell_histogram_dev: call cpf_set_mesh first");
    CPF_REQUIRE(ctx, n >= 0 && weights_dev && (cell || n == 0), CPF_ERR_ARG, "cpf_cell_histogram_dev: bad arguments");
    CPF_HIP(ctx, hipSetDevice(ctx->device));
    if (ctx->d_parentOf) {
        const size_t head = ((size_t)n * 4 + 255) & ~(size_t)255;
        int r = ensureScratch(ctx, head + cpf::histogram_scratch_bytes(ctx->nParent));
        if (r != CPF_OK) return r;
        int32_t* parent = (int32_t*)ctx->scratch;
        CPF_HIP(ctx, cpf::launch_cells_to_parent(ctx->stream, cell, parent, ctx->d_parentOf, n, ctx->host.nCells));
        CPF_HIP(ctx, cpf::cell_histogram(ctx->stream, parent, n, ctx->nParent, scale, weights_dev, (char*)ctx->scratch + head,
                                         ctx->scratchBytes - head));
        return CPF_OK;
    }
    int r = ensureScratch(ctx, cpf::histogram_scratch_bytes(ctx->host.nCells));
    if (r != CPF_OK) return r;
    CPF_HIP(ctx, cpf::cell_histogram(ctx->stream, cell, n, ctx->host.nCells, scale, weights_dev, ctx->scratch,
                                     ctx->scratchBytes));
    return CPF_OK;
}

int cpf_cell_ranges_dev(cpf_context* ctx, const double* weights_dev, int nRanks, int32_t* cellLo_dev) {
    CPF_REQUIRE(ctx, ctx, CPF_ERR_ARG, "null context");
    CPF_REQUIRE(ctx, ctx->haveMesh, CPF_ERR_STATE, "cpf_cell_ranges_dev: call cpf_set_mesh first");
    CPF_REQUIRE(ctx, weights_dev && cellLo_dev && nRanks >= 1 && nRanks <= CPF_MAX_RANKS, CPF_ERR_ARG,
                "cpf_cell_ranges_dev: bad arguments (1 <= nRanks <= CPF_MAX_RANKS)");
    CPF_HIP(ctx, hipSetDevice(ctx->device));
    CPF_HIP(ctx, cpf::cell_ranges(ctx->stream, weights_dev, ctx->nParent, nRanks, cellLo_dev));
    return CPF_OK;
}

int cpf_unpack_arrivals_dev(cpf_context* ctx, double* x, double* y, double* z, int32_t* cell, int64_t* gid,
                            int64_t nStay, const double* recvbuf, int64_t nRecv) {
    CPF_REQUIRE(ctx, ctx, CPF_ERR_ARG, "null context");
    CPF_REQUIRE(ctx, nStay >= 0 && nRecv >= 0 && (nRecv == 0 || (x && y && z && cell && recvbuf)), CPF_ERR_ARG,
                "cpf_unpack_arrivals_dev: bad arguments");
    CPF_HIP(ctx, hipSetDevice(ctx->device));
    CPF_HIP(ctx, cpf::unpack_arrivals(ctx->stream, x, y, z, cell, gid, nStay, recvbuf, nRecv));
    return CPF_OK;
}

int cpf_dev_alloc(cpf_context* ctx, size_t bytes, void** out) {
    CPF_REQUIRE(ctx, ctx && out, CPF_ERR_ARG, "null argument");
    *out = nullptr;
    CPF_HIP(ctx, hipSetDevice(ctx->device));
    CPF_HIP(ctx, hipMalloc(out, std::max<size_t>(bytes, 16)));
    return CPF_OK;
}
int cpf_dev_free(cpf_context* ctx, void* ptr) {
    CPF_REQUIRE(ctx, ctx, CPF_ERR_ARG, "null context");
    if (!ptr) return CPF_OK;
    CPF_HIP(ctx, hipSetDevice(ctx->device));
    CPF_HIP(ctx, hipStreamSynchronize(ctx->stream));
    CPF_HIP(ctx, hipFree(ptr));
    return CPF_OK;
}
int cpf_dev_memset(cpf_context* ctx, void* ptr, int value, size_t bytes) {
    CPF_REQUIRE(ctx, ctx && (ptr || bytes == 0), CPF_ERR_ARG, "null argument");
    CPF_HIP(ctx, hipSetDevice(ctx->device));
    if (bytes) CPF_HIP(ctx, hipMemsetAsync(ptr, value, bytes, ctx->stream));
    return CPF_OK;
}
int cpf_copy_to_device(cpf_context* ctx, void* dst, const void* src, size_t bytes) {
    CPF_REQUIRE(ctx, ctx && ((dst && src) || bytes == 0), CPF_ERR_ARG, "null argument");
    CPF_HIP(ctx, hipSetDevice(ctx->device));
    if (bytes) {
        CPF_HIP(ctx, hipMemcpyAsync(dst, src, bytes, hipMemcpyHostToDevice, ctx->stream));
        CPF_HIP(ctx, hipStreamSynchronize(ctx->stream));
    }
    return CPF_OK;
}
int cpf_copy_to_host(cpf_context* ctx, void* dst, const void* src, size_t bytes) {
    CPF_REQUIRE(ctx, ctx && ((dst && src) || bytes == 0), CPF_ERR_ARG, "null argument");
    CPF_HIP(ctx, hipSetDevice(ctx->device));
    if (bytes) {
        CPF_HIP(ctx, hipMemcpyAsync(dst, src, bytes, hipMemcpyDeviceToHost, ctx->stream));
        CPF_HIP(ctx, hipStreamSynchronize(ctx->stream));
    }
    return CPF_OK;
}

int cpf_copy_dev(cpf_context* ctx, void* dst, const void* src, size_t bytes) {
    CPF_REQUIRE(ctx, ctx && ((dst && src) || bytes == 0), CPF_ERR_ARG, "null argument");
    CPF_HIP(ctx, hipSetDevice(ctx->device));
    if (bytes) CPF_HIP(ctx, hipMemcpyAsync(dst, src, bytes, hipMemcpyDeviceToDevice, ctx->stream));
    return CPF_OK;
}

#define CPF_STAGE_PRE(name, needU)                                                                      \
    CPF_REQUIRE(ctx, ctx, CPF_ERR_ARG, "null context");                                                 \
    CPF_REQUIRE(ctx, ctx->haveMesh, CPF_ERR_STATE, name ": call cpf_set_mesh first");                   \
    CPF_REQUIRE(ctx, !ctx->d_parentOf, CPF_ERR_MESH, name ": the mesh has warped or concave cells decomposed " \
                "into tets (cpf_get_mesh_quality); the reference-layout stages take the mesh's own cells only"); \
    CPF_REQUIRE(ctx, !(needU) || ctx->haveU, CPF_ERR_STATE, name ": call cpf_set_velocity first");      \
    CPF_REQUIRE(ctx, n >= 0, CPF_ERR_ARG, name ": negative particle count");                            \
    CPF_HIP(ctx, hipSetDevice(ctx->device))

int cpf_stage_seed_box(cpf_context* ctx, double* particles, int64_t n, const double lower[3], const double upper[3],
                       int order) {
    CPF_REQUIRE(ctx, ctx, CPF_ERR_ARG, "null context");
    CPF_REQUIRE(ctx, n >= 0 && lower && upper && (particles || n == 0), CPF_ERR_ARG, "cpf_stage_seed_box: bad arguments");
    CPF_HIP(ctx, hipSetDevice(ctx->device));
    int r = ensureScratch(ctx, (size_t)std::max<int64_t>(n, 1) * 24);
    if (r) return r;
    double* x = (double*)ctx->scratch; double* y = x + n; double* z = y + n;
    CPF_HIP(ctx, cpf::launch_seed_box(ctx->stream, x, y, z, 0, n, lower, upper, order));
    CPF_HIP(ctx, cpf::launch_soa_to_aos(ctx->stream, x, y, z, particles, n));
    return CPF_OK;
}
int cpf_stage_locate_initial(cpf_context* ctx, const double* particles, int32_t* ids, int64_t n) {
    CPF_STAGE_PRE("cpf_stage_locate_initial", false);
    CPF_REQUIRE(ctx, n == 0 || (particles && ids), CPF_ERR_ARG, "cpf_stage_locate_initial: null array");
    int r = ensureScratch(ctx, (size_t)std::max<int64_t>(n, 1) * 24);
    if (r) return r;
    double* x = (double*)ctx->scratch; double* y = x + n; double* z = y + n;
    CPF_HIP(ctx, cpf::launch_aos_to_soa(ctx->stream, particles, x, y, z, n));
    CPF_HIP(ctx, cpf::launch_locate_initial(ctx->stream, x, y, z, ids, n, meshView(ctx), gridView(ctx)));
    return CPF_OK;
}
int cpf_stage_count_outside(cpf_context* ctx, const int32_t* ids, int64_t n, int64_t* nNegative) {
    CPF_REQUIRE(ctx, ctx && nNegative && (ids || n == 0) && n >= 0, CPF_ERR_ARG, "cpf_stage_count_outside: bad arguments");
    CPF_HIP(ctx, hipSetDevice(ctx->device));
    unsigned long long* cnt = ctx->d_counters + cpf::kCounterSlots * 4;
    CPF_HIP(ctx, hipMemsetAsync(cnt, 0, 8, ctx->stream));
    CPF_HIP(ctx, cpf::launch_count_negative(ctx->stream, ids, n, cnt));
    unsigned long long h = 0;
    CPF_HIP(ctx, hipMemcpyAsync(&h, cnt, 8, hipMemcpyDeviceToHost, ctx->stream));
    CPF_HIP(ctx, hipStreamSynchronize(ctx->stream));
    *nNegative = (int64_t)h;
    return CPF_OK;
}
int cpf_stage_advect(cpf_context* ctx, double* particles, const int32_t* ids, double* vels, double* disps, double dt,
                     int64_t n) {
    CPF_STAGE_PRE("cpf_stage_advect", true);
    CPF_REQUIRE(ctx, n == 0 || (particles && ids && vels && disps), CPF_ERR_ARG, "cpf_stage_advect: null array");
    CPF_HIP(ctx, cpf::launch_stage_advect(ctx->stream, particles, ids, vels, disps, dt, n, meshView(ctx)));
    return CPF_OK;
}
int cpf_stage_advect_const(cpf_context* ctx, double* particles, const int32_t* ids, const double* vels, double* disps, double dt,
                           int64_t n) {
    CPF_STAGE_PRE("cpf_stage_advect_const", false);
    CPF_REQUIRE(ctx, n == 0 || (particles && ids && vels && disps), CPF_ERR_ARG, "cpf_stage_advect_const: null array");
    CPF_HIP(ctx, cpf::launch_stage_advect_const(ctx->stream, particles, ids, vels, disps, dt, n));
    return CPF_OK;
}
int cpf_set_tets(cpf_context* ctx, const double* positions, int64_t nVerts, const int32_t* tets, int64_t nTets,
                 int tetsPerCell) {
    CPF_REQUIRE(ctx, ctx, CPF_ERR_ARG, "null context");
    CPF_REQUIRE(ctx, ctx->haveMesh, CPF_ERR_STATE, "cpf_set_tets: call cpf_set_mesh first");
    CPF_REQUIRE(ctx, !ctx->d_parentOf, CPF_ERR_MESH, "cpf_set_tets: the mesh has warped or concave cells decomposed into tets "
                "(cpf_get_mesh_quality); the \"VertexVelocity\" mode needs the mesh's own cells (set option \"split_nonplanar\" 0)");
    CPF_REQUIRE(ctx, positions && tets && nVerts > 0 && tetsPerCell > 0, CPF_ERR_ARG, "cpf_set_tets: bad arguments");
    CPF_REQUIRE(ctx, nTets == (int64_t)tetsPerCell * ctx->host.nCells, CPF_ERR_MESH,
                "cpf_set_tets: nTets must be tetsPerCell x nCells (tets in cell order, src/initCuda.H:99-105)");
    for (int64_t k = 0; k < 4 * nTets; ++k)
        CPF_REQUIRE(ctx, tets[k] >= 0 && tets[k] < nVerts, CPF_ERR_MESH, "cpf_set_tets: tet vertex out of range");
    CPF_HIP(ctx, hipSetDevice(ctx->device));
    CPF_HIP(ctx, hipStreamSynchronize(ctx->stream));
    freeDev(ctx->d_tetPos); freeDev(ctx->d_tets); freeDev(ctx->d_vertVel); freeDev(ctx->d_vertCone); freeDev(ctx->d_vertApex);
    ctx->haveVertVel = false;
    CPF_HIP(ctx, hipMalloc((void**)&ctx->d_tetPos, (size_t)nVerts * 24));
    CPF_HIP(ctx, hipMalloc((void**)&ctx->d_tets, (size_t)nTets * 16));
    CPF_HIP(ctx, hipMalloc((void**)&ctx->d_vertVel, (size_t)nVerts * 24));
    CPF_HIP(ctx, hipMemcpyAsync(ctx->d_tetPos, positions, (size_t)nVerts * 24, hipMemcpyHostToDevice, ctx->stream));
    CPF_HIP(ctx, hipMemcpyAsync(ctx->d_tets, tets, (size_t)nTets * 16, hipMemcpyHostToDevice, ctx->stream));
    CPF_HIP(ctx, hipStreamSynchronize(ctx->stream));
    ctx->nTetVerts = nVerts; ctx->nTets = nTets; ctx->tetsPerCell = tetsPerCell;
    ctx->vertConeWhy = tetFanDefect(positions, tets, ctx->host.nCells, tetsPerCell);
    if (ctx->vertConeWhy.empty()) {
        CPF_HIP(ctx, hipMalloc((void**)&ctx->d_vertCone, (size_t)nTets * 256));
        CPF_HIP(ctx, hipMalloc((void**)&ctx->d_vertApex, (size_t)ctx->host.nCells * 32));
        CPF_HIP(ctx, cpf::launch_vertex_cone_tables(ctx->stream, ctx->d_tetPos, ctx->d_tets, nTets, tetsPerCell, ctx->d_vertCone, ctx->d_vertApex));
        CPF_HIP(ctx, hipStreamSynchronize(ctx->stream));
    }
    return CPF_OK;
}
int cpf_set_vertex_velocity(cpf_context* ctx, const double* vertexU, int64_t nVerts) {
    CPF_REQUIRE(ctx, ctx && vertexU, CPF_ERR_ARG, "null argument");
    CPF_REQUIRE(ctx, ctx->d_tets, CPF_ERR_STATE, "cpf_set_vertex_velocity: call cpf_set_tets first");
    CPF_REQUIRE(ctx, nVerts == ctx->nTetVerts, CPF_ERR_ARG, "cpf_set_vertex_velocity: one velocity per tet-mesh vertex");
    CPF_HIP(ctx, hipSetDevice(ctx->device));
    CPF_HIP(ctx, hipMemcpyAsync(ctx->d_vertVel, vertexU, (size_t)nVerts * 24, hipMemcpyHostToDevice, ctx->stream));
    if (ctx->d_vertCone) CPF_HIP(ctx, cpf::launch_vertex_record_velocity(ctx->stream, ctx->d_tets, ctx->d_vertVel, ctx->nTets, ctx->d_vertCone));
    CPF_HIP(ctx, hipStreamSynchronize(ctx->stream));
    ctx->haveVertVel = true;
    return CPF_OK;
}
int cpf_stage_advect_vertex(cpf_context* ctx, double* particles, const int32_t* ids, double* vels, double* disps,
                            double dt, int64_t n) {
    CPF_STAGE_PRE("cpf_stage_advect_vertex", false);
    CPF_REQUIRE(ctx, ctx->haveVertVel && ctx->nTets == (int64_t)ctx->tetsPerCell * ctx->host.nCells, CPF_ERR_STATE,
                "cpf_stage_advect_vertex: call cpf_set_tets and cpf_set_vertex_velocity (for the current mesh) first");
    CPF_REQUIRE(ctx, n == 0 || (particles && ids && vels && disps), CPF_ERR_ARG, "cpf_stage_advect_vertex: null array");
    CPF_HIP(ctx, cpf::launch_stage_advect_vertex(ctx->stream, particles, ids, vels, disps, dt, n, ctx->d_tetPos, ctx->d_tets,
                                                 ctx->tetsPerCell, ctx->d_vertVel, ctx->vertexFast ? ctx->d_vertCone : nullptr, ctx->d_vertApex));
    return CPF_OK;
}
int cpf_stage_brownian(cpf_context* ctx, const double* particles, double* disps, double dt, int64_t n, double D,
                       uint32_t step) {
    CPF_REQUIRE(ctx, ctx, CPF_ERR_ARG, "null context");
    CPF_REQUIRE(ctx, n >= 0 && (n == 0 || (particles && disps)) && D >= 0.0, CPF_ERR_ARG, "cpf_stage_brownian: bad arguments");
    CPF_HIP(ctx, hipSetDevice(ctx->device));
    CPF_HIP(ctx, cpf::launch_stage_brownian(ctx->stream, particles, disps, dt, n, D, step, ctx->seed));
    return CPF_OK;
}
int cpf_stage_locate(cpf_context* ctx, const double* particles, const double* disps, int32_t* ids, int64_t n) {
    CPF_STAGE_PRE("cpf_stage_locate", false);
    CPF_REQUIRE(ctx, n == 0 || (particles && disps && ids), CPF_ERR_ARG, "cpf_stage_locate: null array");
    CPF_HIP(ctx, cpf::launch_stage_locate(ctx->stream, particles, disps, ids, n, meshView(ctx)));
    return CPF_OK;
}
int cpf_stage_reflect(cpf_context* ctx, int32_t* ids, double* particles, double* vels, double* disps, int64_t n) {
    CPF_STAGE_PRE("cpf_stage_reflect", false);
    CPF_REQUIRE(ctx, n == 0 || (particles && disps && ids && vels), CPF_ERR_ARG, "cpf_stage_reflect: null array");
    CPF_HIP(ctx, cpf::launch_stage_reflect(ctx->stream, ids, particles, vels, disps, n, meshView(ctx)));
    return CPF_OK;
}
int cpf_stage_move(cpf_context* ctx, double* particles, double* disps, int64_t n) {
    CPF_REQUIRE(ctx, ctx, CPF_ERR_ARG, "null context");
    CPF_REQUIRE(ctx, n >= 0 && (n == 0 || (particles && disps)), CPF_ERR_ARG, "cpf_stage_move: bad arguments");
    CPF_HIP(ctx, hipSetDevice(ctx->device));
    CPF_HIP(ctx, cpf::launch_stage_move(ctx->stream, particles, disps, n));
    return CPF_OK;
}

int cpf_write_vtu_wait(cpf_context* ctx) {
    CPF_REQUIRE(ctx, ctx, CPF_ERR_ARG, "null context");
    if (!ctx->writerLive) return CPF_OK;
    ctx->writer.join();
    ctx->writerLive = false;
    {
        std::lock_guard<std::mutex> lk(g_mutex);
        auto& v = g_writers.live;
        v.erase(std::remove(v.begin(), v.end(), ctx), v.end());
    }
    const int r = ctx->writerStatus;
    ctx->writerStatus = CPF_OK;
    if (r != CPF_OK && r != CPF_WARN_NAN) return fail(ctx, r, "cpf_write_vtu_async: the frame could not be written");
    return r;
}

int cpf_write_vtu_async(cpf_context* ctx, const char* path, double* totalKE) {
    CPF_REQUIRE(ctx, ctx && path, CPF_ERR_ARG, "null argument");
    int r = cpf_write_vtu_wait(ctx);
    if (r != CPF_OK && r != CPF_WARN_NAN) return r;
    CPF_REQUIRE(ctx, ctx->n > 0, CPF_ERR_STATE, "cpf_write_vtu_async: no particles");
    CPF_HIP(ctx, hipSetDevice(ctx->device));
    const size_t n = (size_t)ctx->n;
    auto al = [](size_t b) { return (b + 255) & ~(size_t)255; };
    const size_t offC = al(n * 32), offV = offC + al(n * 4), need = offV + al(n * 32);
    if (!ctx->ioStream) {
        CPF_HIP(ctx, hipStreamCreateWithFlags(&ctx->ioStream, hipStreamNonBlocking));
        CPF_HIP(ctx, hipEventCreateWithFlags(&ctx->evSnap, hipEventDisableTiming));
        CPF_HIP(ctx, hipEventCreateWithFlags(&ctx->evCopied, hipEventDisableTiming));
    }
    if (need > ctx->snapBytes) {
        if (ctx->snapDev) { (void)hipFree(ctx->snapDev); ctx->snapDev = nullptr; }
        if (ctx->snapHost) { (void)hipHostFree(ctx->snapHost); ctx->snapHost = nullptr; }
        ctx->snapBytes = 0;
        const size_t want = need + need / 8;
        hipError_t e = hipMalloc(&ctx->snapDev, want);
        if (e == hipSuccess) e = hipHostMalloc(&ctx->snapHost, want, hipHostMallocDefault);
        if (e != hipSuccess) {
            if (ctx->snapDev) { (void)hipFree(ctx->snapDev); ctx->snapDev = nullptr; }
            return fail(ctx, e == hipErrorOutOfMemory ? CPF_ERR_NOMEM : CPF_ERR_HIP, std::string("cpf_write_vtu_async: snapshot buffers: ") + hipGetErrorString(e));
        }
        ctx->snapBytes = want;
    }
    char* d = (char*)ctx->snapDev;
    CPF_HIP(ctx, cpf::launch_pack_by_gid(ctx->stream, ctx->x, ctx->y, ctx->z, ctx->cell, ctx->gid, ctx->vel, (double*)d, (int32_t*)(d + offC),
                                         (double*)(d + offV), ctx->n));
    if (ctx->d_parentOf)
        CPF_HIP(ctx, cpf::launch_cells_to_parent(ctx->stream, (const int32_t*)(d + offC), (int32_t*)(d + offC), ctx->d_parentOf, ctx->n,
                                                 ctx->host.nCells));
    CPF_HIP(ctx, hipEventRecord(ctx->evSnap, ctx->stream));
    CPF_HIP(ctx, hipStreamWaitEvent(ctx->ioStream, ctx->evSnap, 0));
    CPF_HIP(ctx, hipMemcpyAsync(ctx->snapHost, ctx->snapDev, need, hipMemcpyDeviceToHost, ctx->ioStream));
    CPF_HIP(ctx, hipEventRecord(ctx->evCopied, ctx->ioStream));
    const std::string file(path);
    { std::lock_guard<std::mutex> lk(g_mutex); g_writers.live.push_back(ctx); }
    ctx->writerLive = true;
    ctx->keReady = false;
    const bool binary = ctx->vtuBinary;
    ctx->writer = std::thread([ctx, file, n, binary, offC, offV] {
        (void)hipSetDevice(ctx->device);
        const hipError_t e = hipEventSynchronize(ctx->evCopied);
        const char* h = (const char*)ctx->snapHost;
        const double* xyzw = (const double*)h; const int32_t* cell = (const int32_t*)(h + offC); const double* vel = (const double*)(h + offV);
        double total = 0.0;
        if (e == hipSuccess)
            for (size_t i = 0; i < n; ++i) total += 0.5 * (vel[4 * i] * vel[4 * i] + vel[4 * i + 1] * vel[4 * i + 1] + vel[4 * i + 2] * vel[4 * i + 2]);
        { std::lock_guard<std::mutex> lk(ctx->keMutex); ctx->frameKE = total; ctx->keReady = true; }
        ctx->keCv.notify_all();
        ctx->writerStatus = e != hipSuccess ? CPF_ERR_HIP
                                            : (binary ? cpf_write_vtu_arrays_binary : cpf_write_vtu_arrays)(file.c_str(), (int64_t)n, xyzw, cell, vel, nullptr);
    });
    if (!totalKE) return CPF_OK;
    std::unique_lock<std::mutex> lk(ctx->keMutex);
    ctx->keCv.wait(lk, [ctx] { return ctx->keReady; });
    *totalKE = ctx->frameKE;
    return std::isnan(ctx->frameKE) ? CPF_WARN_NAN : CPF_OK;
}

int cpf_timing_enable(cpf_context* ctx, int on) {
    CPF_REQUIRE(ctx, ctx, CPF_ERR_ARG, "null context");
    ctx->timing = on != 0;
    return CPF_OK;
}

int cpf_timing_read(cpf_context* ctx, int64_t* launches, double* total_ms) {
    CPF_REQUIRE(ctx, ctx && launches && total_ms, CPF_ERR_ARG, "null argument");
    CPF_HIP(ctx, hipSetDevice(ctx->device));
    CPF_HIP(ctx, hipStreamSynchronize(ctx->stream));
    double tot = 0.0;
    for (auto& p : ctx->events) {
        float ms = 0.f;
        CPF_HIP(ctx, hipEventElapsedTime(&ms, p.first, p.second));
        tot += (double)ms;
        ctx->eventPool.push_back(p.first); ctx->eventPool.push_back(p.second);
    }
    *launches = (int64_t)ctx->events.size();
    *total_ms = tot;
    ctx->events.clear();
    return CPF_OK;
}

int cpf_timing_poll(cpf_context* ctx, int64_t* launches, double* total_ms) {
    CPF_REQUIRE(ctx, ctx && launches && total_ms, CPF_ERR_ARG, "null argument");
    CPF_HIP(ctx, hipSetDevice(ctx->device));
    double tot = 0.0;
    size_t done = 0;
    for (; done < ctx->events.size(); ++done) {
        auto& p = ctx->events[done];
        const hipError_t q = hipEventQuery(p.second);
        if (q == hipErrorNotReady) break;
        CPF_HIP(ctx, q);
        float ms = 0.f;
        CPF_HIP(ctx, hipEventElapsedTime(&ms, p.first, p.second));
        tot += (double)ms;
        ctx->eventPool.push_back(p.first); ctx->eventPool.push_back(p.second);
    }
    ctx->events.erase(ctx->events.begin(), ctx->events.begin() + (std::ptrdiff_t)done);
    *launches = (int64_t)done;
    *total_ms = tot;
    return CPF_OK;
}

}
```

cudaparticlesfoam_amd/csrc/cpf_device.h:

```cpp
#pragma once
#include <hip/hip_runtime.h>

#include <cstdint>
#include <type_traits>

#include "cpf.h"
#include "cpf_internal.h"

namespace cpf {

constexpr int kBlock = 256;
constexpr int kCounterSlots = 1024;

struct MeshView {
    const int32_t* cellOff;
    const double4* planes;
    const int32_t* nbr;
    const int32_t* groupOff;
    const int32_t* groupNbr;
    const double4* U;
    const double4* cellRec;
    const double4* boxRec;
    int32_t nCells;
    int32_t allHex;
    int32_t zPairLast;
    int32_t zSide0;
    int32_t zThin;
    int32_t mixed;
};

struct GridView {
    double origin[3], invBin[3], lo[3], hi[3];
    int32_t dims[3];
    const int32_t* binOff;
    const int32_t* binCells;
};

constexpr size_t kStreamGrabBytes = 2 * 256 * 16 * sizeof(unsigned);
constexpr int kStreamHitSpillDoubles = 3 * 64;
struct StreamState {
    unsigned* d_grab = nullptr;
    double* d_hitSpill = nullptr;
    int hitSpillWaves = 0;
    int parity = 0;
    int numCU = 256;
    int tilesPerChunk = 0;
    int wavesPerCU = 0;
    int coopMaxCells = 0;
    int lookup = -1;
    double tailFraction = -1.0;
    int debug = 0;
    const volatile unsigned long long* occupiedHost = nullptr;
    int densityLookup = 0;
    bool flatField = false;
    int flat = 1;
    int flatZ = 1;
};

constexpr int kCoopMaxCells = 1 << 24;
constexpr int kFusedCoopCycles = 1 << 30;
struct VertexField;

struct StepPlan {
    enum Kernel { kGeneric = 0, kFixed = 1, kFixedScalar = 2, kCoop = 3, kStream = 4, kAhead = 5, kVertex, kStreamVertex };
    Kernel kernel = kGeneric;
    bool brown = false, reflect = false, storeVel = false, stats = false;
    int lookup = -1;
    bool cone = false;
    bool stamped() const { return kernel == kStream || kernel == kStreamVertex; }
    bool flat() const { return kernel == kStream && (lookup == 8 || lookup == 9); }
};
StepPlan plan_step(const MeshView& m, const StreamState& ss, int variant, const VertexField* vf, int64_t n, int nCyc, double D,
                   unsigned flags, bool stats);
hipError_t launch_step(const StepPlan& p, hipStream_t st, double* x, double* y, double* z, int32_t* cell, const int64_t* gid,
                       double* vel, int64_t n, double dt, double D, uint32_t step0, int nCyc, uint32_t seed, const MeshView& m,
                       unsigned long long* counters, const VertexField* vf, StreamState& ss, bool zSettled, hipEvent_t evStart,
                       hipEvent_t evStop);
hipError_t launch_step_stream(const StepPlan& p, hipStream_t st, double* x, double* y, double* z, int32_t* cell, const int64_t* gid,
                              double* vel, int64_t n, double dt, double sigma, uint32_t step0, int nCyc, uint32_t seed,
                              const MeshView& m, unsigned long long* counters, const VertexField* vf, StreamState& ss, bool zSettled,
                              hipEvent_t evStart, hipEvent_t evStop);
hipError_t launch_step_ahead(const StepPlan& p, hipStream_t st, double* x, double* y, double* z, int32_t* cell, int64_t n, double dt,
                             const MeshView& m, unsigned long long* counters, StreamState& ss, double* dbg);
template <class F>
decltype(auto) with_bools(F&& f) { return f(); }
template <class F, class... Bs>
decltype(auto) with_bools(F&& f, bool b, Bs... bs) {
    if (b) return with_bools([&](auto... c) -> decltype(auto) { return f(std::true_type{}, c...); }, bs...);
    return with_bools([&](auto... c) -> decltype(auto) { return f(std::false_type{}, c...); }, bs...);
}

hipError_t launch_locate_initial(hipStream_t st, const double* x, const double* y, const double* z, int32_t* cell,
                                 int64_t n, const MeshView& m, const GridView& g);
hipError_t launch_seed_box(hipStream_t st, double* x, double* y, double* z, int64_t first, int64_t n,
                           const double lower[3], const double upper[3], int order);
hipError_t launch_iota64(hipStream_t st, int64_t* p, int64_t n, int64_t first);
hipError_t launch_unpack_xyz(hipStream_t st, const double* xyz, double* x, double* y, double* z, int64_t n);
hipError_t launch_pack_by_gid(hipStream_t st, const double* x, const double* y, const double* z, const int32_t* cell,
                              const int64_t* gid, const double* vel, double* xyzw, int32_t* cellOut, double* velOut,
                              int64_t n);
hipError_t launch_count_negative(hipStream_t st, const int32_t* cell, int64_t n, unsigned long long* out);
hipError_t launch_build_cell_records(hipStream_t st, const double4* planes, const int32_t* nbr, const double4* U,
                                     double4* rec, int64_t nCells);
hipError_t launch_build_cell_records_mixed(hipStream_t st, const int32_t* cellOff, const double4* planes, const int32_t* nbr,
                                           const double4* U, const int32_t* recB, double4* rec, int64_t nCells);
hipError_t launch_update_record_velocity(hipStream_t st, const double4* U, double4* rec, double* box, int64_t nCells);
hipError_t launch_u3_to_u4(hipStream_t st, const double* u3, double4* u4, int64_t nCells, unsigned long long* zFlag = nullptr);
hipError_t launch_gather_parent_u3(hipStream_t st, const double* uParent, const int32_t* parentOf, double* uDerived, int64_t nDerived);
hipError_t launch_cells_to_parent(hipStream_t st, const int32_t* in, int32_t* out, const int32_t* parentOf, int64_t n, int64_t nDerived);

hipError_t launch_stage_advect(hipStream_t st, double* P, const int32_t* ids, double* vels, double* disps, double dt,
                               int64_t n, const MeshView& m);
hipError_t launch_stage_advect_const(hipStream_t st, double* P, const int32_t* ids, const double* vels, double* disps, double dt,
                                     int64_t n);
hipError_t launch_stage_advect_vertex(hipStream_t st, double* P, const int32_t* ids, double* vels, double* disps, double dt,
                                      int64_t n, const double* pos, const int32_t* tets, int tetsPerCell,
                                      const double* vertVel, const double* cone, const double* apex);
hipError_t launch_vertex_cone_tables(hipStream_t st, const double* pos, const int32_t* tets, int64_t nTets, int tetsPerCell, double* cone,
                                     double* apex);
hipError_t launch_vertex_record_velocity(hipStream_t st, const int32_t* tets, const double* vel, int64_t nTets, double* cone);
hipError_t launch_stage_brownian(hipStream_t st, const double* P, double* disps, double dt, int64_t n, double D,
                                 uint32_t step, uint32_t seed);
hipError_t launch_stage_locate(hipStream_t st, const double* P, const double* disps, int32_t* ids, int64_t n,
                               const MeshView& m);
hipError_t launch_stage_reflect(hipStream_t st, int32_t* ids, double* P, double* vels, double* disps, int64_t n,
                                const MeshView& m);
hipError_t launch_stage_move(hipStream_t st, double* P, double* disps, int64_t n);
hipError_t launch_aos_to_soa(hipStream_t st, const double* P, double* x, double* y, double* z, int64_t n);
hipError_t launch_soa_to_aos(hipStream_t st, const double* x, const double* y, const double* z, double* P, int64_t n);

size_t sort_scratch_bytes(int64_t n, int endBit);
hipError_t sort_by_cell(hipStream_t st, double* x, double* y, double* z, int32_t* cell, int64_t* gid, double* vel3,
                        int64_t n, int endBit, const float* cellBox, const int* subBits, const int* subOrder,
                        void* scratch, size_t scratchBytes, double* ox = nullptr, double* oy = nullptr, double* oz = nullptr,
                        int32_t* ocell = nullptr, int64_t* ogid = nullptr, unsigned long long* occupied = nullptr,
                        const int32_t* rank = nullptr, int method = 1);

size_t handoff_scratch_bytes(int64_t n, int nRanks);
hipError_t pack_leavers(hipStream_t st, double* x, double* y, double* z, int32_t* cell, int64_t* gid, int64_t n,
                        const int32_t* cellLo, int nRanks, int myRank, double* sendbuf, int64_t sendCapacity,
                        int64_t* counts, int64_t* nStay, void* scratch, size_t scratchBytes);
size_t histogram_scratch_bytes(int64_t nCells);
hipError_t cell_histogram(hipStream_t st, const int32_t* cell, int64_t n, int64_t nCells, double scale, double* weights,
                          void* scratch, size_t scratchBytes);
hipError_t cell_ranges(hipStream_t st, const double* weights, int64_t nCells, int nRanks, int32_t* cellLo);
hipError_t unpack_arrivals(hipStream_t st, double* x, double* y, double* z, int32_t* cell, int64_t* gid,
                           int64_t nStay, const double* recvbuf, int64_t nRecv);
constexpr int kOutputDoubles = 8;
hipError_t pack_output(hipStream_t st, const double* x, const double* y, const double* z, const int32_t* cell,
                       const int64_t* gid, const double* vel3, double* rec, int64_t n);
hipError_t scatter_output(hipStream_t st, const double* rec, int64_t nRec, int64_t nGlobal, double* xyzw, int32_t* cellOut,
                          double* velOut, unsigned long long* bad);
hipError_t sum_rows(hipStream_t st, const double* rows, int nRows, size_t count, double* out);

}
```

cudaparticlesfoam_amd/csrc/cpf_stream.hip:

```cpp
#include "cpf_stream_ops.h"

#include <hip/hip_ext.h>

#include <type_traits>

namespace cpf {

#ifndef CPF_STREAM_SLOTS
#define CPF_STREAM_SLOTS 6
#endif
#ifndef CPF_STREAM_SLOTS_FIXED
#define CPF_STREAM_SLOTS_FIXED 9
#endif
#ifndef CPF_STREAM_WAVES
#define CPF_STREAM_WAVES 7
#endif
constexpr int kStreamSlots = CPF_STREAM_SLOTS;
constexpr int kStreamSlotsFixed = CPF_STREAM_SLOTS_FIXED;
constexpr int kSlotStride = 8;
static_assert(kStreamSlots >= 4 && kStreamSlots <= 32 && kStreamSlotsFixed >= 4 && kStreamSlotsFixed <= 32, "slots");
#ifndef CPF_STREAM_GATHER_LANES
#define CPF_STREAM_GATHER_LANES 32
#endif
constexpr int kStreamGatherLanes = CPF_STREAM_GATHER_LANES;
#ifndef CPF_STREAM_PAIRED
#define CPF_STREAM_PAIRED 0
#endif
#ifndef CPF_STREAM_INROUND
#define CPF_STREAM_INROUND 0
#endif
#ifndef CPF_STREAM_HIT_POOL
#define CPF_STREAM_HIT_POOL 40
#endif
constexpr int kVertexTets = 12;
#ifndef CPF_VERTEX_BLOCKS
#define CPF_VERTEX_BLOCKS 4
#endif
#ifndef CPF_VERTEX_PICK_UNROLL
#define CPF_VERTEX_PICK_UNROLL 12
#endif
constexpr int kVertexBlocks = CPF_VERTEX_BLOCKS;
constexpr int kStreamSparsePerCell = 8;
constexpr int kSitOut = INT32_MIN + 7;

struct StreamKernArgs {
    double *x, *y, *z; int32_t* cell; const int64_t* gid; double* vel; int64_t n; double dt, sigma; uint32_t step0; int nCyc;
    uint32_t seed; MeshView m; unsigned long long* counters; StreamArgs sa;
};
static_assert(offsetof(StreamKernArgs, x) == 0 && offsetof(StreamKernArgs, cell) == 24, "kernarg_cloud_ptrs reads bytes 0..31");
constexpr int kKernArgHitSpill = (int)(offsetof(StreamKernArgs, sa) + offsetof(StreamArgs, hitSpill));
constexpr int kKernArgGid = (int)offsetof(StreamKernArgs, gid), kKernArgSigma = (int)offsetof(StreamKernArgs, sigma);
constexpr int kKernArgStep0 = (int)offsetof(StreamKernArgs, step0), kKernArgSeed = (int)offsetof(StreamKernArgs, seed);
#ifndef CPF_STREAM_BROWN_KERNARG
#define CPF_STREAM_BROWN_KERNARG 1
#endif

#ifndef CPF_STREAM_L1_ZERO_SKIP
#define CPF_STREAM_L1_ZERO_SKIP 1
#endif
#ifndef CPF_STREAM_LAZY_USED
#define CPF_STREAM_LAZY_USED 1
#endif
#ifndef CPF_STREAM_BOX_SPARSE
#define CPF_STREAM_BOX_SPARSE 1
#endif
#ifndef CPF_STREAM_FLAT_KICK
#define CPF_STREAM_FLAT_KICK 0
#endif
#ifndef CPF_STREAM_FLAT_ZERO_SKIP
#define CPF_STREAM_FLAT_ZERO_SKIP 0
#endif
#ifndef CPF_STREAM_FLAT_Z
#define CPF_STREAM_FLAT_Z 1
#endif
#ifndef CPF_STREAM_SLOTS_BOX
#define CPF_STREAM_SLOTS_BOX 9
#endif
#ifndef CPF_STREAM_SLOTS_BOX_B
#define CPF_STREAM_SLOTS_BOX_B 12
#endif
#ifndef CPF_STREAM_WAVES_BOX_B
#define CPF_STREAM_WAVES_BOX_B 6
#endif
#ifndef CPF_STREAM_WAVES_BOX
#define CPF_STREAM_WAVES_BOX 6
#endif
#ifndef CPF_STREAM_WAVES_B1
#define CPF_STREAM_WAVES_B1 5
#endif
#ifndef CPF_STREAM_WAVES_L2
#define CPF_STREAM_WAVES_L2 6
#endif
#ifndef CPF_STREAM_WAVES_B0
#define CPF_STREAM_WAVES_B0 7
#endif
#ifndef CPF_STREAM_HIT_POOL_B0
#define CPF_STREAM_HIT_POOL_B0 18
#endif
#ifndef CPF_STREAM_WAVES_FLAT
#define CPF_STREAM_WAVES_FLAT CPF_STREAM_WAVES
#endif
template <bool BROWNIAN, bool STORE_VEL, bool STATS, int LOOKUP>
struct StreamOccupancy {
    static constexpr bool kMixed = LOOKUP == 2 || LOOKUP == 3 || LOOKUP == 5 || LOOKUP == 11;
    static constexpr int waves = (STORE_VEL || STATS) ? 1 : (LOOKUP == 4 ? (BROWNIAN ? 4 : 5) : (BROWNIAN ? (kMixed ? 5 : ((LOOKUP == 6 || LOOKUP == 11) ? CPF_STREAM_WAVES_BOX_B : (LOOKUP == 1 ? CPF_STREAM_WAVES_B1 : CPF_STREAM_WAVES_B0))) : (LOOKUP == 2 ? CPF_STREAM_WAVES_L2 : ((kMixed && LOOKUP != 11) ? 6 : ((LOOKUP == 6 || LOOKUP == 11) ? CPF_STREAM_WAVES_BOX : (LOOKUP == 8 ? CPF_STREAM_WAVES_FLAT : CPF_STREAM_WAVES))))));
};

template <bool BROWNIAN, bool REFLECT, bool STORE_VEL, bool STATS, int LOOKUP, bool VERTEX>
__device__ __forceinline__ void stream_body(
    const int64_t* __restrict__ gid, double* __restrict__ vel, int64_t n, double dt, double sigma, uint32_t step0,
    int nCyc, uint32_t seed, const MeshView& m, unsigned long long* __restrict__ counters, const StreamArgs& sa, const VertexField& vf) {
#ifndef CPF_STREAM_SLOTS_BROWN
#define CPF_STREAM_SLOTS_BROWN 10
#endif
    constexpr int NS = (LOOKUP == 0 || LOOKUP == 5 || LOOKUP == 8) ? kStreamSlots : ((LOOKUP == 6 || LOOKUP == 11) ? (BROWNIAN ? CPF_STREAM_SLOTS_BOX_B : CPF_STREAM_SLOTS_BOX) : (BROWNIAN && LOOKUP == 1 ? CPF_STREAM_SLOTS_BROWN : kStreamSlotsFixed));
    constexpr bool BOX = LOOKUP == 6 || LOOKUP == 11;
    constexpr int kStride = BOX ? 4 : kSlotStride;
    constexpr unsigned kRecBytes = 32u * kStride;
    constexpr unsigned ALL = NS == 32 ? 0xFFFFFFFFu : ((1u << NS) - 1u);
    __shared__ double4 slots[NS][kStride];
    __shared__ unsigned sCnt[4];
#ifndef CPF_STREAM_HIT_REGS_L2
#define CPF_STREAM_HIT_REGS_L2 0
#endif
    constexpr bool HIT_IN_REGS = !BROWNIAN && (LOOKUP != 2 || CPF_STREAM_HIT_REGS_L2);
    constexpr bool kInRound = CPF_STREAM_INROUND == 2 || (CPF_STREAM_INROUND == 1 && BROWNIAN);
    static_assert(!(kInRound && (LOOKUP == 2 || LOOKUP == 3 || LOOKUP == 5 || LOOKUP == 11)), "in-round reflection knows neither face groups nor two-record cells");
    constexpr int kPool = HIT_IN_REGS ? 1 : ((LOOKUP == 2 || LOOKUP == 3 || LOOKUP == 5 || LOOKUP == 11) ? 16 : ((BROWNIAN && LOOKUP == 0) ? CPF_STREAM_HIT_POOL_B0 : CPF_STREAM_HIT_POOL));
    __shared__ double sLane[3][64];
    __shared__ double sPool[3][kPool];
    __shared__ unsigned sPoolUsed;
    __shared__ double sPre[BROWNIAN ? 288 : 224];
    __shared__ double sCone[VERTEX ? kVertexBlocks : 1][VERTEX ? kVertexTets * 10 : 1];
    double(*sE)[64] = sLane;
    const int lane = threadIdx.x;
    const unsigned ul = threadIdx.x;
    const unsigned preBase = uniform32(lds_addr(sPre));
    const unsigned slotBase = uniform32(lds_addr(slots));
    const int tpc = sa.tilesPerChunk;
    constexpr bool LOOKUP_FIXED = LOOKUP != 0 && LOOKUP != 5 && LOOKUP != 8;
    constexpr bool FLAT = LOOKUP == 8 || LOOKUP == 9;
    const bool zKeep = FLAT && CPF_STREAM_FLAT_Z != 0 && sa.zSettled != 0;
    constexpr bool mixed = LOOKUP == 2 || LOOKUP == 3 || LOOKUP == 5 || LOOKUP == 11;
    constexpr bool bigCells = LOOKUP == 2;
    constexpr int kGatherAhead = LOOKUP == 4 ? 3 : 0;
    const bool zFold = !BOX && BROWNIAN && REFLECT && m.zThin != 0;
    const bool zLast = !FLAT && !BROWNIAN && m.zPairLast != 0;
    const bool flatKick = zFold && m.zSide0 != 0;
    const unsigned nTiles = (unsigned)((n + 63) >> 6);
    const unsigned nFull = (unsigned)(n >> 6), nTail = (unsigned)n & 63u;
    const unsigned big = sa.bigChunks;
    const unsigned nChunks = big + (nTiles - big * (unsigned)tpc);
    auto chunk_first = [&](unsigned c) -> unsigned {
        return c < big ? c * (unsigned)tpc : big * (unsigned)tpc + (c - big);
    };
    auto chunk_tiles = [&](unsigned c, unsigned firstTile) -> int {
        if (c >= nChunks) return 0;
        const unsigned k = nTiles - firstTile;
        const unsigned want = c < big ? (unsigned)tpc : 1u;
        return (int)(k < want ? k : want);
    };
    auto chunk_of = [&](unsigned j) -> unsigned {
        const unsigned long long c = (unsigned long long)(blockIdx.x & (kStreamGroups - 1)) + (unsigned long long)kStreamGroups * j;
        return c < (unsigned long long)nChunks ? (unsigned)c : nChunks;
    };
    StepStats st = {0, 0, 0, 0};
#ifdef CPF_STREAM_TIMELINE
    const uint64_t tl0 = __builtin_amdgcn_s_memrealtime();
    unsigned tlTiles = 0, tlRounds = 0;
    unsigned tlWaitRec = 0, tlWaitEnd = 0, tlMissRounds = 0;
    unsigned long long* const tlH = (!STORE_VEL && vel != nullptr && (sa.debug & 4)) ? reinterpret_cast<unsigned long long*>(vel) + 8 * 16384 : nullptr;
    unsigned tlVis = 0, tlRoundIdx = 0;
#endif

    for (unsigned k = blockIdx.x; k < (unsigned)kStreamGroups; k += gridDim.x)
        if (lane == 0) sa.grabNext[k * kStreamCounterStride] = 0u;
    const unsigned grp = blockIdx.x & (kStreamGroups - 1);
    unsigned* const myGrab = sa.grab + grp * kStreamCounterStride;

    auto prefetch = [&](unsigned t, const CloudPtrs& cp) __attribute__((always_inline)) -> int {
        double* const x = cp.x; double* const y = cp.y; double* const z = cp.z; int32_t* const cell = cp.cell;
        t = uniform32(t);
        const int64_t b = (int64_t)t * 64;
        unsigned ul = threadIdx.x;
        asm volatile("" : "+v"(ul));
        if (t < nFull) {
            const char* s1 = (ul < 32u ? reinterpret_cast<const char*>(x + b) : reinterpret_cast<const char*>(y + b)) + (ul & 31u) * 16u;
            glds16(s1, preBase);
            if (zKeep) {
                if (ul < 16u) glds16(reinterpret_cast<const char*>(cell + b) + ul * 16u, preBase + 1024u);
            } else if (ul < 48u) {
                const char* s2 = ul < 32u ? reinterpret_cast<const char*>(z + b) + ul * 16u
                                          : reinterpret_cast<const char*>(cell + b) + (ul - 32u) * 16u;
                glds16(s2, preBase + 1024u);
            }
            if (BROWNIAN) {
                const int64_t* const g = CPF_STREAM_BROWN_KERNARG ? static_cast<const int64_t*>(kernarg_pointer<kKernArgGid>()) : gid;
                if (g != nullptr) {
                    if (ul < 32u) glds16(reinterpret_cast<const char*>(g + b) + ul * 16u, preBase + 1792u);
                    return 3;
                }
            }
            return 2;
        }
        const unsigned lim = nTail - 1u;
        const unsigned l = ul < lim ? ul : lim;
        if (zKeep) {
            const double vx = (x + b)[l], vy = (y + b)[l];
            const int vc = (cell + b)[l];
            sPre[ul] = vx; sPre[64 + ul] = vy;
            reinterpret_cast<int*>(sPre + 128)[ul] = vc;
        } else {
        const double vx = (x + b)[l], vy = (y + b)[l], vz = (z + b)[l];
        const int vc = (cell + b)[l];
        sPre[ul] = vx; sPre[64 + ul] = vy; sPre[128 + ul] = vz;
        reinterpret_cast<int*>(sPre + 192)[ul] = vc;
        }
        if (BROWNIAN) {
            const int64_t* const g = CPF_STREAM_BROWN_KERNARG ? static_cast<const int64_t*>(kernarg_pointer<kKernArgGid>()) : gid;
            if (g != nullptr) reinterpret_cast<int64_t*>(sPre + 224)[ul] = (g + b)[l];
        }
        return 0;
    };

    unsigned got0 = 0;
    if (lane == 0) got0 = grab_sync(myGrab);
    const unsigned chunk0 = chunk_of(uniform32(got0));
    if (chunk_tiles(chunk0, chunk_first(chunk0)) > 0) {
        int tagv = -1;
        unsigned fifo = 0;

        unsigned tile = chunk_first(chunk0);
        int tilesLeft = chunk_tiles(chunk0, tile);
        (void)prefetch(tile, kernarg_cloud_ptrs());
        wait_vmcnt<0>();

        bool havePrev = false;
        unsigned rtile = 0;
        double rvx = 0, rvy = 0, rvz = 0;
        bool ralive = false;
        int rc = 0;
        unsigned rlim = 63;

        for (;;) {
            tile = uniform32(tile);
            const unsigned plim = tile < nFull ? 63u : nTail - 1u;
            double px = sPre[ul], py = sPre[64 + ul], pz = 0.0;
            int pc;
            if (zKeep) pc = reinterpret_cast<const int*>(sPre + 128)[ul];
            else { pz = sPre[128 + ul]; pc = reinterpret_cast<const int*>(sPre + 192)[ul]; }
            uint64_t pid = 0;
            if (BROWNIAN) {
                const bool haveIds = (CPF_STREAM_BROWN_KERNARG ? kernarg_pointer<kKernArgGid>() : (void*)gid) != nullptr;
                pid = haveIds ? (uint64_t) reinterpret_cast<const int64_t*>(sPre + 224)[ul] : (uint64_t)tile * 64 + ul;
            }
            if (ul > plim || pc < 0) pc = CPF_CELL_FROZEN;

            int cur = pc;
            int key2 = 0, carNext = 0, carBest = -1;
            double carDT = 2.0;
            D3 S_ = {px, py, pz}, v = {0, 0, 0};
            const uint64_t id = pid;

            unsigned ntile = 0;
            int ntilesLeft = 0;

            auto hook = [&](const D3& prev) __attribute__((always_inline)) -> int {
                int younger = 0;
                __builtin_amdgcn_sched_barrier(0);
                if (tilesLeft > 1) {
                    ntile = tile + 1;
                    ntilesLeft = tilesLeft - 1;
                } else {
                    unsigned got = 0;
                    if (lane == 0) got = grab_sync(myGrab);
                    const unsigned nxt = chunk_of(uniform32(got));
                    ntile = chunk_first(nxt);
                    ntilesLeft = chunk_tiles(nxt, ntile);
                }
                const CloudPtrs cp = kernarg_cloud_ptrs();
                double* const x = cp.x; double* const y = cp.y; double* const z = cp.z; int32_t* const cell = cp.cell;
                if (havePrev && !(sa.debug & 1)) {
                    const int64_t b = (int64_t)uniform32(rtile) * 64;
                    if (STORE_VEL && ralive) {
                        double* vv = vel + 3 * b;
                        async_store(vv, ul * 24u, rvx); async_store(vv + 1, ul * 24u, rvy); async_store(vv + 2, ul * 24u, rvz);
                    }
                    if (ul <= rlim) {
                        async_store(x + b, ul * 8u, prev.x); async_store(y + b, ul * 8u, prev.y);
                        if (!zKeep) async_store(z + b, ul * 8u, prev.z);
                        async_store(cell + b, ul * 4u, rc);
                    }
                    younger += zKeep ? 3 : 4;
                }
                if (ntilesLeft > 0 && !(sa.debug & 2)) younger += prefetch(ntile, cp);
                __builtin_amdgcn_sched_barrier(0);
                return younger;
            };

            bool busy = false;
            bool zUnclear = false;
            int token = INT32_MIN, h = 0, j = 0;
            int hitAt = -1;
            D3 hitReg = {0, 0, 0};
            auto park_hit = [&](const D3& Hp) __attribute__((always_inline)) {
                if (HIT_IN_REGS) { hitReg = Hp; return; }
                if (hitAt < 0) hitAt = (int)atomicAdd(&sPoolUsed, 1u);
                if (hitAt < kPool) { sPool[0][hitAt] = Hp.x; sPool[1][hitAt] = Hp.y; sPool[2][hitAt] = Hp.z; }
                else {
                    double* sp = static_cast<double*>(kernarg_pointer<kKernArgHitSpill>()) + (size_t)blockIdx.x * kStreamHitSpillDoubles;
                    async_store(sp, ul * 8u, Hp.x); async_store(sp + 64, ul * 8u, Hp.y); async_store(sp + 128, ul * 8u, Hp.z);
                }
            };

            auto cycle_begin = [&](int c) __attribute__((always_inline)) {
                if (cur < 0) cur = CPF_CELL_FROZEN;
                busy = cur >= 0;
                token = INT32_MIN; h = 0; j = 0;
                if (bigCells) key2 = 0;
                if (!HIT_IN_REGS && REFLECT) { hitAt = -1; if (lane == 0) sPoolUsed = 0u; }
                zUnclear = false;
                if (STATS && busy) ++st.steps;
                if (VERTEX) {
                    bool slow = busy;
#if defined(CPF_VERTEX_AB) && CPF_VERTEX_AB == 1
                    if (busy) { const double4 u = m.U[cur]; v = {u.x, u.y, u.z}; slow = false; }
#endif
                    if (vf.tetsPerCell == kVertexTets) {
                        unsigned long long todo = ballot64(slow);
                        while (todo != 0ull) {
                            int myBlock = -1;
                            __syncthreads();
#pragma unroll
                            for (int q = 0; q < kVertexBlocks; ++q) {
                                if (todo != 0ull) {
                                    const int ck = __builtin_amdgcn_readlane(cur, __ffsll((long long)todo) - 1);
                                    const bool mine = slow && cur == ck;
                                    if (mine) myBlock = q;
                                    if (lane < 5 * kVertexTets) {
                                        const int tk = lane / 5, piece = lane - 5 * tk;
                                        const double2 row = reinterpret_cast<const double2*>(vf.cone + kConeDoubles * ((int64_t)ck * kVertexTets + tk))[piece];
                                        reinterpret_cast<double2*>(&sCone[q][0] + 10 * tk)[piece] = row;
                                    }
                                    todo &= ~ballot64(mine);
                                }
                            }
                            __syncthreads();
                            if (myBlock >= 0) {
                                const double4 ap = vf.apex[cur];
                                const D3 A = {ap.x, ap.y, ap.z};
                                const D3 r = {S_.x - A.x, S_.y - A.y, S_.z - A.z};
                                int cand = 0;
                                double candMin = -1e300;
                                const double* blk = &sCone[myBlock][0];
#pragma unroll CPF_VERTEX_PICK_UNROLL
                                for (int k = 0; k < kVertexTets; ++k) {
                                    const double2* g = reinterpret_cast<const double2*>(blk + 10 * k);
                                    const double2 g01 = g[0], g23 = g[1], g45 = g[2], g67 = g[3], g89 = g[4];
                                    const double cb = fma(g23.x, r.z, fma(g01.y, r.y, g01.x * r.x)), cc = fma(g45.y, r.z, fma(g45.x, r.y, g23.y * r.x));
                                    const double cd = fma(g89.x, r.z, fma(g67.y, r.y, g67.x * r.x));
                                    const double mm = fmin(cb, fmin(cc, cd));
                                    if (mm > candMin) { candMin = mm; cand = k; }
                                }
#if defined(CPF_VERTEX_AB) && CPF_VERTEX_AB == 2
                                { const double4 u = m.U[cur]; v = {u.x + 1e-300 * cand, u.y, u.z}; slow = false; }
#else
                                D3 vv;
                                if (vertex_velocity_in_tet(vf, S_, A, (int64_t)cur * kVertexTets + cand, vv)) { v = vv; slow = false; }
#endif
                            }
                        }
                    }
                    if (slow) (void)vertex_velocity(vf, S_, cur, v);
                }
            };

            auto round = [&](bool hookDue, bool cycleStart, int c) __attribute__((always_inline)) {
#ifdef CPF_STREAM_TIMELINE
                ++tlRounds;
                bool tlSat = false;
#endif
                const unsigned long long busyMask = ballot64(busy);
                const D3 Epre = {sE[0][lane], sE[1][lane], sE[2][lane]};
                const int lk = (bigCells && key2 != 0) ? key2 : cur;
                int myslot = -1;
                unsigned used = 0;
                unsigned long long missLanes = busyMask;
                if (LOOKUP_FIXED) {
                    const int cell0 = __builtin_amdgcn_readlane(lk, __ffsll((long long)busyMask) - 1);
                    const unsigned long long in0 = __builtin_amdgcn_uicmp((unsigned)lk, (unsigned)cell0, 32 ) & busyMask;
                    if (in0 == busyMask) {
                        const unsigned long long hitTag = __builtin_amdgcn_uicmp((unsigned)tagv, (unsigned)cell0, 32 ) & ALL;
                        if (hitTag != 0ull) {
                            myslot = __ffsll((long long)hitTag) - 1;
                            used = (unsigned)hitTag;
                            missLanes = 0ull;
                        }
                    } else {
#if CPF_STREAM_LAZY_USED
                        unsigned long long eqs[NS];
#pragma unroll
                        for (int k = 0; k < NS; ++k) {
                            const int tk = __builtin_amdgcn_readlane(tagv, k);
                            eqs[k] = __builtin_amdgcn_uicmp((unsigned)lk, (unsigned)tk, 32 );
                            asm("v_cndmask_b32_e64 %0, %1, %2, %3" : "=v"(myslot) : "v"(myslot), "n"(k), "s"(eqs[k]));
                        }
                        missLanes = ballot64(myslot < 0) & busyMask;
                        if (missLanes != 0ull) {
#pragma unroll
                            for (int k = 0; k < NS; ++k) used |= ((eqs[k] & busyMask) != 0ull ? 1u : 0u) << k;
                        }
#else
#pragma unroll
                        for (int k = 0; k < NS; ++k) {
                            const int tk = __builtin_amdgcn_readlane(tagv, k);
                            const unsigned long long eqK = __builtin_amdgcn_uicmp((unsigned)lk, (unsigned)tk, 32 );
                            const unsigned long long inK = eqK & busyMask;
                            asm("v_cndmask_b32_e64 %0, %1, %2, %3" : "=v"(myslot) : "v"(myslot), "n"(k), "s"(eqK));
                            used |= (inK != 0ull ? 1u : 0u) << k;
                            missLanes &= ~inK;
                        }
#endif
                    }
                } else {
                    unsigned long long todo = busyMask;
                    missLanes = 0ull;
                    while (todo != 0ull) {
                        const int leader = __ffsll((long long)todo) - 1;
                        const int ck = __builtin_amdgcn_readlane(lk, leader);
                        const bool mine = lk == ck;
                        const unsigned long long same = ballot64(mine) & busyMask;
                        const unsigned long long hitTag = __builtin_amdgcn_uicmp((unsigned)tagv, (unsigned)ck, 32 );
                        if (hitTag != 0ull) {
                            const int sl = __ffsll((long long)hitTag) - 1;
                            used |= 1u << sl;
                            if (mine) myslot = sl;
                        } else {
                            missLanes |= same;
                        }
                        todo &= ~same;
                    }
                }
                int nJobs = 0;
                if (missLanes != 0ull) {
#define CPF_JOB(J)                                                                                          \
                    if (missLanes != 0ull && used != ALL) {                                                 \
                        const int leader = __ffsll((long long)missLanes) - 1;                               \
                        const int ck = __builtin_amdgcn_readlane(lk, leader);                               \
                        const unsigned cand = ~used & ALL;                                                  \
                        const unsigned hi = cand & (ALL << fifo) & ALL;                                     \
                        const int victim = __ffs((int)(hi ? hi : cand)) - 1;                                \
                        fifo = (unsigned)(victim + 1) == (unsigned)NS ? 0u : (unsigned)(victim + 1);          \
                        used |= 1u << victim;                                                               \
                        if (lane == victim) tagv = ck;                                                      \
                        const bool mine = lk == ck;                                                         \
                        if (mine) myslot = victim;                                                          \
                        missLanes &= ~ballot64(mine);                                                       \
                        if (ul < kRecBytes / 16u)                                                            \
                            glds16(reinterpret_cast<const char*>(BOX ? m.boxRec : m.cellRec) + (int64_t)ck * kRecBytes + ul * 16u,  \
                                   uniform32(slotBase + (unsigned)victim * kRecBytes));                     \
                        nJobs = J + 1;                                                                      \
                    }
                    CPF_JOB(0) CPF_JOB(1) CPF_JOB(2) CPF_JOB(3)
                    if (LOOKUP_FIXED) { CPF_JOB(4) CPF_JOB(5) CPF_JOB(6) CPF_JOB(7) }
#undef CPF_JOB
                }
                int younger = 0;
                if (hookDue) younger = hook(Epre);
                if (BROWNIAN && cycleStart && busy) {
                    uint32_t kStep0 = step0, kSeed = seed;
                    if (CPF_STREAM_BROWN_KERNARG) kernarg_u32_pair<kKernArgStep0, kKernArgSeed>(kStep0, kSeed);
                    const D3 xi = normal3(id, kStep0 + (uint32_t)c, kSeed);
                    sE[0][lane] = xi.x; sE[1][lane] = xi.y; sE[2][lane] = xi.z;
                }
#ifdef CPF_STREAM_TIMELINE
                const uint64_t tlw0 = __builtin_amdgcn_s_memrealtime();
#endif
                if (nJobs != 0) {
                    if (younger >= 7) wait_vmcnt<7>();
                    else if (younger == 6) wait_vmcnt<6>();
                    else if (younger == 5) wait_vmcnt<5>();
                    else if (younger >= 4) wait_vmcnt<4>();
                    else if (younger == 3) wait_vmcnt<3>();
                    else if (younger >= 2) wait_vmcnt<2>();
                    else wait_vmcnt<0>();
#ifdef CPF_STREAM_TIMELINE
                    tlWaitRec += (unsigned)(__builtin_amdgcn_s_memrealtime() - tlw0); ++tlMissRounds;
#endif
                }
                const bool gatherRound = __popcll(missLanes) >= kStreamGatherLanes;
                auto advect = [&](const double4* rec) __attribute__((always_inline)) -> D3 {
                    D3 Pn;
                    if (VERTEX) {
                        Pn = {S_.x + dt * v.x, S_.y + dt * v.y, S_.z + dt * v.z};
                    } else {
                        double4 u;
                        if (BOX) { const double2 uxy = reinterpret_cast<const double2*>(rec)[5]; u = {uxy.x, uxy.y, reinterpret_cast<const double*>(rec)[12], 0.0}; }
                        else u = rec[6];
                        v = {u.x, u.y, u.z};
                        Pn = axpy(dt, v, S_);
                    }
                    D3 disp = {Pn.x - S_.x, Pn.y - S_.y, Pn.z - S_.z};
                    if (BROWNIAN) {
                        const D3 xi = {sE[0][lane], sE[1][lane], sE[2][lane]};
                        disp = axpy(CPF_STREAM_BROWN_KERNARG ? kernarg_f64<kKernArgSigma>() : sigma, xi, disp);
                    }
                    D3 E = {S_.x + disp.x, S_.y + disp.y, S_.z + disp.z};
                    if (BROWNIAN && REFLECT && zFold) {
                        bool clear;
                        const int nb = fold_z(E.z, rec[BOX ? 0 : 4], rec[BOX ? 0 : 5], clear);
                        zUnclear |= ballot64(!clear) != 0ull;
                        if (STATS) st.refl += nb;
                        if (STORE_VEL && (nb & 1)) v.z = -v.z;
                    }
                    sE[0][lane] = E.x; sE[1][lane] = E.y; sE[2][lane] = E.z;
                    return E;
                };
                if (busy) {
                    int next, outSlot = 0;
                    double4 wallPlane;
                    const bool needAdvect = token == INT32_MIN && !(bigCells && key2 != 0);
                    D3 E = S_;
                    if (!needAdvect) E = Epre;
                    bool hdrCell = false;
                    if (bigCells && myslot >= 0) hdrCell = *reinterpret_cast<const int*>(&slots[0][0] + myslot * kSlotStride + 7) == kBigCellMark;
                    if (myslot >= 0 && !(bigCells && hdrCell)) {
                        const double4* rec = &slots[0][0] + myslot * kStride;
                        if (needAdvect) E = advect(rec);
                        bool twoRec = false;
                        int recB = 0;
                        const bool second0 = key2 != 0;
                        if (bigCells) {
                            const int2 cont = reinterpret_cast<const int2*>(rec + 7)[3];
                            twoRec = !second0 && cont.x == kTwoRecMark;
                            recB = cont.y;
                        }
                        bool again;
                        do {
                            again = false;
                            if (bigCells) {
                                const D3 P0 = S_;
                                const D3 Pd = {E.x - P0.x, E.y - P0.y, E.z - P0.z};
                                double dTm = second0 ? carDT : 2.0;
                                int nx = second0 ? carNext : cur, bs = second0 ? carBest : -1;
                                trace_lds6_record<!BROWNIAN, mixed>(P0, Pd, rec, token, second0 ? 6 : 0, dTm, nx, bs);
                                if (twoRec) {
                                    carDT = dTm; carNext = nx; carBest = bs;
                                    key2 = recB;
                                    next = kSitOut;
                                } else {
                                    key2 = 0;
                                    if (bs >= 0) { S_ = axpy(dTm, Pd, P0); outSlot = bs; }
                                    next = nx;
                                    if (STATS) ++st.hops;
                                }
                            } else {
                            if (BOX) next = trace_box<!BROWNIAN, mixed>(S_, E, cur, rec, token, outSlot);
                            else if (FLAT) next = trace_lds4_flat<(CPF_STREAM_FLAT_ZERO_SKIP != 0)>(S_, E, cur, rec, token, outSlot);
                            else if (CPF_STREAM_FLAT_KICK && BROWNIAN && !mixed && flatKick && !zUnclear)
                            next = trace_lds4_flat_z<false>(S_, E, cur, rec, token, outSlot);
                            else
                            next = (CPF_STREAM_PAIRED && LOOKUP_FIXED && !BROWNIAN && !mixed) ? trace_lds6_paired(S_, E, cur, rec, token, outSlot, zLast)
                                                                : trace_lds6<(!BROWNIAN && (CPF_STREAM_L1_ZERO_SKIP || LOOKUP != 1)), mixed>(S_, E, cur, rec, token, outSlot, zLast, zFold && !zUnclear);
                            if (STATS) ++st.hops;
                            }
                            if (REFLECT && next < 0 && !(mixed && is_group(next))) {
                                if (bigCells && lk != cur) {
                                    if (outSlot >= 6) wallPlane = rec[outSlot - 6];
                                    else {
                                        wallPlane = m.planes[m.cellOff[cur] + outSlot];
                                        asm volatile("" : "+v"(wallPlane.x), "+v"(wallPlane.y), "+v"(wallPlane.z), "+v"(wallPlane.w));
                                    }
                                } else if (BOX) wallPlane = box_wall_plane(rec, outSlot);
                                else wallPlane = rec[outSlot];
                                asm volatile("" ::: "memory");
                                E = {sE[0][lane], sE[1][lane], sE[2][lane]};
                                if (kInRound) {
                                    park_hit(S_);
                                    if (STATS) ++st.refl;
                                    const D3 nn = {wallPlane.x, wallPlane.y, wallPlane.z};
                                    const double sd = dot3(wallPlane, E) - wallPlane.w;
                                    E = axpy(-2.0 * sd, nn, E);
                                    sE[0][lane] = E.x; sE[1][lane] = E.y; sE[2][lane] = E.z;
                                    v = axpy(-2.0 * dot3(wallPlane, v), nn, v);
                                    token = next;
                                    h = 0;
                                    if (++j == kMaxReflect) { busy = false; next = cur; }
                                    else again = true;
                                }
                            }
                        } while (again);
                    } else {
                        next = kSitOut;
                        if (gatherRound || (bigCells && hdrCell)) {
                            const double4* rec = BOX ? m.boxRec + 4 * (int64_t)cur : m.cellRec + 8 * (int64_t)cur;
                            if (needAdvect) E = advect(rec);
                            int gS0 = 0;
                            bool gBig = false;
                            if (LOOKUP_FIXED && bigCells) {
                                const int4 hdr = *reinterpret_cast<const int4*>(rec + 7);
                                const int2 cont = reinterpret_cast<const int2*>(rec + 7)[3];
                                gBig = hdr.x == kBigCellMark || cont.x == kTwoRecMark;
                                if (gBig) {
                                    gS0 = m.cellOff[cur];
                                    next = trace_csr(S_, E, cur, m.planes, m.nbr, gS0, m.cellOff[cur + 1] - gS0, token, outSlot);
                                    rec = m.planes + gS0;
                                    key2 = 0;
                                }
                            }
                            if (BOX) next = trace_box<false, mixed>(S_, E, cur, rec, token, outSlot);
                            else if (!gBig)
                            next = trace_fixed<6, false, mixed, kGatherAhead>(S_, E, cur, rec, reinterpret_cast<const int32_t*>(rec + 7), token, outSlot, 0);
                            if (STATS) ++st.hops;
                            if (REFLECT && next < 0) {
                                wallPlane = BOX ? box_wall_plane(rec, outSlot) : rec[outSlot];
                                asm volatile("" : "+v"(wallPlane.x), "+v"(wallPlane.y), "+v"(wallPlane.z), "+v"(wallPlane.w));
                            }
                        }
                    }
                    if (mixed && next != kSitOut && is_group(next)) next = resolve_group(next, S_, m.cellOff, m.planes, m.groupOff, m.groupNbr);
#ifdef CPF_STREAM_TIMELINE
                    if (next == kSitOut) tlSat = true; else ++tlVis;
#endif
                    const bool ends = next == cur;
                    const bool wall = next < 0 && next != kSitOut;
                    const bool cross = next >= 0 && !ends;
                    if (wall) {
                        if (!REFLECT) j = kMaxReflect;
                        else {
                            park_hit(S_);
                            if (STATS) ++st.refl;
                            const D3 nn = {wallPlane.x, wallPlane.y, wallPlane.z};
                            const double sd = dot3(wallPlane, E) - wallPlane.w;
                            E = axpy(-2.0 * sd, nn, E);
                            sE[0][lane] = E.x; sE[1][lane] = E.y; sE[2][lane] = E.z;
                            v = axpy(-2.0 * dot3(wallPlane, v), nn, v);
                            h = 0;
                            ++j;
                        }
                    }
                    token = cross ? cur : (wall ? next : token);
                    cur = cross ? next : cur;
                    h += cross ? 1 : 0;
                    busy = !(ends || (cross && h == kMaxHops) || (wall && j >= kMaxReflect));
                }
#ifdef CPF_STREAM_TIMELINE
                {
                    const unsigned nb = (unsigned)__popcll(busyMask), ns = (unsigned)__popcll(ballot64(tlSat));
                    const unsigned r = tlRoundIdx < 15u ? tlRoundIdx : 15u;
                    if (tlH != nullptr && lane == 0) {
                        atomicAdd(&tlH[r * 65u + nb], 1ull); atomicAdd(&tlH[16 * 65 + r], (unsigned long long)ns);
                        atomicAdd(&tlH[16 * 65 + 16 + 256 + r], (unsigned long long)nJobs);
                    }
                    ++tlRoundIdx;
                }
#endif
            };

            auto cycle_end = [&]() __attribute__((always_inline)) {
                if (cur >= 0) {
                    const D3 E = {sE[0][lane], sE[1][lane], sE[2][lane]};
                    if (REFLECT && j != 0) {
                        D3 hit;
                        if (HIT_IN_REGS) hit = hitReg;
                        else if (hitAt < kPool) hit = {sPool[0][hitAt], sPool[1][hitAt], sPool[2][hitAt]};
                        else load3_sync(static_cast<const double*>(kernarg_pointer<kKernArgHitSpill>()) + (size_t)blockIdx.x * kStreamHitSpillDoubles,
                                        ul * 8u, hit.x, hit.y, hit.z);
                        S_ = {hit.x + (E.x - hit.x), hit.y + (E.y - hit.y), hit.z + (E.z - hit.z)};
                    } else S_ = E;
                    if (j >= kMaxReflect) { cur = CPF_CELL_LOST; if (STATS) ++st.lost; }
                }
            };

            if (nCyc > 0) {
                for (int c = 0; c < nCyc; ++c) {
                    cycle_begin(c);
#ifdef CPF_STREAM_TIMELINE
                    tlVis = 0; tlRoundIdx = 0;
#endif
                    bool hookDue = c == 0, cycleStart = true;
#ifdef CPF_STREAM_CAP_TEST
                    int capRounds = 0, capLimit = CPF_STREAM_CAP_TEST;
                    asm volatile("" : "+s"(capLimit));
                    do { round(hookDue, cycleStart, c); hookDue = false; cycleStart = false; ++capRounds; } while (ballot64(busy) != 0ull && capRounds < capLimit);
                    const bool capDropped = busy;
                    const D3 capKeep = S_;
                    const int capCur = cur;
#else
                    do { round(hookDue, cycleStart, c); hookDue = false; cycleStart = false; } while (ballot64(busy) != 0ull);
#endif
#ifdef CPF_STREAM_TIMELINE
                    {
                        unsigned mx = tlVis;
                        for (int off = 32; off > 0; off >>= 1) { const unsigned o = (unsigned)__shfl_xor((int)mx, off, 64); mx = o > mx ? o : mx; }
                        const unsigned r = tlRoundIdx < 15u ? tlRoundIdx : 15u, iv = mx < 15u ? mx : 15u;
                        if (tlH != nullptr && lane == 0) atomicAdd(&tlH[16 * 65 + 16 + r * 16u + iv], 1ull);
                    }
#endif
                    cycle_end();
#ifdef CPF_STREAM_CAP_TEST
                    if (capDropped) { S_ = capKeep; cur = capCur; }
#endif
                }
            } else {
                const D3 prev = {sE[0][lane], sE[1][lane], sE[2][lane]};
                (void)hook(prev);
            }

#ifdef CPF_STREAM_TIMELINE
            const uint64_t tle0 = __builtin_amdgcn_s_memrealtime();
#endif
            wait_vmcnt<0>();
#ifdef CPF_STREAM_TIMELINE
            tlWaitEnd += (unsigned)(__builtin_amdgcn_s_memrealtime() - tle0);
            ++tlTiles;
#endif
            rtile = tile; havePrev = true;
            sE[0][lane] = S_.x; sE[1][lane] = S_.y; sE[2][lane] = S_.z;
            if (STORE_VEL) { rvx = v.x; rvy = v.y; rvz = v.z; ralive = pc >= 0; }
            rc = cur;
            rlim = plim;
            if (ntilesLeft <= 0) break;
            tile = ntile; tilesLeft = ntilesLeft;
        }
        {
            const int64_t b = (int64_t)rtile * 64;
            const CloudPtrs cp = kernarg_cloud_ptrs();
            double* const x = cp.x; double* const y = cp.y; double* const z = cp.z; int32_t* const cell = cp.cell;
            const double rx = sE[0][lane], ry = sE[1][lane], rz = sE[2][lane];
            if (ul <= rlim) {
                (x + b)[ul] = rx; (y + b)[ul] = ry;
                if (!zKeep) (z + b)[ul] = rz;
                (cell + b)[ul] = rc;
            }
            if (STORE_VEL && ralive) {
                double* vv = vel + 3 * b;
                vv[3 * ul] = rvx; vv[3 * ul + 1] = rvy; vv[3 * ul + 2] = rvz;
            }
        }
    }
#ifdef CPF_STREAM_TIMELINE
    if (!STORE_VEL && vel != nullptr && lane == 0) {
        uint64_t* o = reinterpret_cast<uint64_t*>(vel) + 8 * (uint64_t)blockIdx.x;
        o[0] = tl0; o[1] = __builtin_amdgcn_s_memrealtime(); o[2] = tlTiles; o[3] = tlRounds;
        o[4] = tlWaitRec; o[5] = tlWaitEnd; o[6] = tlMissRounds; o[7] = 0;
    }
#endif
    if (STATS) flush_stats(st, counters, sCnt);
}

template <bool BROWNIAN, bool REFLECT, bool STORE_VEL, bool STATS, int LOOKUP>
__global__ __launch_bounds__(64, (StreamOccupancy<BROWNIAN, STORE_VEL, STATS, LOOKUP>::waves)) void step_kernel_stream(
    double* __restrict__ , double* __restrict__ , double* __restrict__ , int32_t* __restrict__ ,
    const int64_t* __restrict__ gid, double* __restrict__ vel, int64_t n, double dt, double sigma, uint32_t step0,
    int nCyc, uint32_t seed, MeshView m, unsigned long long* __restrict__ counters, StreamArgs sa) {
    stream_body<BROWNIAN, REFLECT, STORE_VEL, STATS, LOOKUP, false>(gid, vel, n, dt, sigma, step0, nCyc, seed, m, counters, sa, VertexField{});
}

#ifndef CPF_STREAM_WAVES_VERTEX
#define CPF_STREAM_WAVES_VERTEX 4
#endif
template <bool BROWNIAN, bool REFLECT, bool STORE_VEL, bool STATS, int LOOKUP>
__global__ __launch_bounds__(64, ((STORE_VEL || STATS) ? 1 : CPF_STREAM_WAVES_VERTEX)) void step_kernel_stream_vertex(
    double* __restrict__ , double* __restrict__ , double* __restrict__ , int32_t* __restrict__ ,
    const int64_t* __restrict__ gid, double* __restrict__ vel, int64_t n, double dt, double sigma, uint32_t step0,
    int nCyc, uint32_t seed, MeshView m, unsigned long long* __restrict__ counters, StreamArgs sa, VertexField vf) {
    stream_body<BROWNIAN, REFLECT, STORE_VEL, STATS, LOOKUP, true>(gid, vel, n, dt, sigma, step0, nCyc, seed, m, counters, sa, vf);
}

template <bool B, bool R_, bool SV, bool ST, int LF, bool VX = false>
static hipError_t launch_stream_inst(hipStream_t st, double* x, double* y, double* z, int32_t* cell, const int64_t* gid,
                                     double* vel, int64_t n, double dt, double sigma, uint32_t step0, int nCyc,
                                     uint32_t seed, const MeshView& m, unsigned long long* counters, StreamState& ss,
                                     const VertexField* vf, bool settled, hipEvent_t evStart, hipEvent_t evStop) {
    static int wavesPerCU = 0;
    if (wavesPerCU == 0) {
        int nb = 0;
        hipError_t e;
        if constexpr (VX) e = hipOccupancyMaxActiveBlocksPerMultiprocessor(&nb, step_kernel_stream_vertex<B, R_, SV, ST, LF>, 64, 0);
        else e = hipOccupancyMaxActiveBlocksPerMultiprocessor(&nb, step_kernel_stream<B, R_, SV, ST, LF>, 64, 0);
        if (e != hipSuccess) return e;
        wavesPerCU = nb < 1 ? 1 : (nb > 32 ? 32 : nb);
    }
    const int64_t nTiles = (n + 63) >> 6;
    if (nTiles >= ((int64_t)1 << 31)) return hipErrorInvalidValue;
    const int64_t slotsOnChip = (int64_t)((ss.wavesPerCU > 0 && !VX) ? ss.wavesPerCU : wavesPerCU) * ss.numCU;
    int tpc = ss.tilesPerChunk > 0 ? ss.tilesPerChunk : ((LF == 0 || LF == 5 || LF == 8) ? 4 : 3);
    const double tailFraction = ss.tailFraction >= 0.0 ? ss.tailFraction : ((LF == 0 || LF == 5 || LF == 8) ? 0.1 : 0.2);
    while (tpc > 1 && nTiles / tpc < 4 * slotsOnChip) tpc = tpc > 2 ? tpc - 1 : 1;
    int64_t bigChunks = (int64_t)((double)(nTiles / tpc) * (1.0 - tailFraction));
    if (tpc == 1 || bigChunks < 0) bigChunks = 0;
    const int64_t nChunks = bigChunks + (nTiles - bigChunks * tpc);
    int64_t R = slotsOnChip / kStreamGroups;
    const int64_t need = (nChunks + kStreamGroups - 1) / kStreamGroups;
    if (R > need) R = need;
    if (R < 1) R = 1;
    unsigned* cur = ss.d_grab + (size_t)(ss.parity & 1) * kStreamGroups * kStreamCounterStride;
    unsigned* nxt = ss.d_grab + (size_t)((ss.parity & 1) ^ 1) * kStreamGroups * kStreamCounterStride;
    if (R * kStreamGroups > ss.hitSpillWaves) R = ss.hitSpillWaves / kStreamGroups;
    if (R < 1 || ss.d_hitSpill == nullptr) return hipErrorInvalidValue;
    const bool zSettled = (LF == 8 || LF == 9) && !VX && settled && ss.flatZ != 0;
    StreamArgs sa = {cur, nxt, (int)R, tpc, (unsigned)bigChunks, ss.debug, ss.d_hitSpill, zSettled ? 1 : 0};
    if constexpr (VX) {
        if (vf == nullptr) return hipErrorInvalidValue;
        if (evStart != nullptr && evStop != nullptr)
            hipExtLaunchKernelGGL((step_kernel_stream_vertex<B, R_, SV, ST, LF>), dim3((unsigned)(R * kStreamGroups)), dim3(64), 0, st, evStart,
                                  evStop, 0, x, y, z, cell, gid, vel, n, dt, sigma, step0, nCyc, seed, m, counters, sa, *vf);
        else
        hipLaunchKernelGGL((step_kernel_stream_vertex<B, R_, SV, ST, LF>), dim3((unsigned)(R * kStreamGroups)), dim3(64), 0, st, x, y, z, cell,
                           gid, vel, n, dt, sigma, step0, nCyc, seed, m, counters, sa, *vf);
        return stream_launch_done(st, ss);
    } else {
    if (evStart != nullptr && evStop != nullptr)
        hipExtLaunchKernelGGL((step_kernel_stream<B, R_, SV, ST, LF>), dim3((unsigned)(R * kStreamGroups)), dim3(64), 0, st, evStart,
                              evStop, 0, x, y, z, cell, gid, vel, n, dt, sigma, step0, nCyc, seed, m, counters, sa);
    else
    hipLaunchKernelGGL((step_kernel_stream<B, R_, SV, ST, LF>), dim3((unsigned)(R * kStreamGroups)), dim3(64), 0, st, x, y, z, cell,
                       gid, vel, n, dt, sigma, step0, nCyc, seed, m, counters, sa);
    return stream_launch_done(st, ss);
    }
}

static int stream_lookup_mode(int64_t n, const MeshView& m, const StreamState& ss, bool brown, bool vertex) {
    int64_t cells = m.nCells;
    if (ss.densityLookup && ss.occupiedHost != nullptr) {
        const int64_t occ = (int64_t)ss.occupiedHost[0], live = (int64_t)ss.occupiedHost[1];
        if (occ > 0 && occ <= cells && live > 0 && live <= 2 * n && n <= 2 * live) cells = occ;
    }
    if (vertex) return n < 128 * cells ? 1 : 0;
    if (m.mixed == 1 && m.boxRec != nullptr && m.zThin == 0 && ss.lookup < 0) return 11;
    if (m.mixed) return m.mixed == 2 ? 2 : ((ss.lookup >= 0 ? ss.lookup == 0 : n >= 128 * cells) ? 5 : 3);
    const bool box = m.boxRec != nullptr && m.zThin == 0;
    if (ss.lookup >= 0) return (ss.lookup == 6 && !box) ? 1 : ss.lookup;
    if (box && CPF_STREAM_BOX_SPARSE) return 6;
    if (n < kStreamSparsePerCell * cells) return 4;
    const bool flat = !brown && ss.flat && ss.flatField && m.zSide0 != 0;
    if (n < 128 * cells) return flat ? 9 : 1;
    return flat ? 8 : 0;
}

StepPlan plan_step(const MeshView& m, const StreamState& ss, int variant, const VertexField* vf, int64_t n, int nCyc, double D,
                   unsigned flags, bool stats) {
    StepPlan p;
    p.brown = D > 0.0;
    p.reflect = (flags & CPF_STEP_NO_REFLECT) == 0;
    p.storeVel = (flags & CPF_STEP_STORE_VEL) != 0;
    p.stats = stats;
    const int coopMaxCells = (ss.coopMaxCells <= 0 || ss.coopMaxCells > kCoopMaxCells) ? kCoopMaxCells : ss.coopMaxCells;
    if (!m.allHex) {
        const bool wantsStream = variant == kVariantAuto || variant == kVariantStream || variant == kVariantCoop;
        variant = (m.mixed && m.cellRec && wantsStream) ? kVariantStream : kVariantGeneric;
    } else {
        if (variant == kVariantAuto)
            variant = !(nCyc >= kFusedCoopCycles && m.nCells <= coopMaxCells) ? kVariantStream : kVariantCoop;
        if (variant == kVariantCoop && m.nCells > coopMaxCells) variant = kVariantStream;
#ifndef CPF_EXPERIMENTS
        if (variant == kVariantFixed || variant == kVariantFixedScalar) variant = kVariantCoop;
        if (variant == kVariantAhead) variant = kVariantStream;
#endif
    }
    if (vf != nullptr) {
        p.cone = vf->cone != nullptr;
        const bool streams = p.cone && vf->tetsPerCell == 12 && m.mixed == 0 && m.cellRec != nullptr && variant == kVariantStream;
        p.kernel = streams ? StepPlan::kStreamVertex : StepPlan::kVertex;
        if (streams) p.lookup = stream_lookup_mode(n, m, ss, p.brown, true);
        return p;
    }
    if (variant == kVariantAhead && (p.brown || p.storeVel || nCyc != 1)) variant = kVariantStream;
    p.kernel = (StepPlan::Kernel)variant;
    if (variant == kVariantStream) p.lookup = stream_lookup_mode(n, m, ss, p.brown, false);
    return p;
}

template <int... L, class F>
static hipError_t with_lookup(int lookup, F&& f) {
    hipError_t e = hipErrorInvalidValue;
    (void)((lookup == L && ((e = f(std::integral_constant<int, L>{})), true)) || ...);
    return e;
}
hipError_t launch_step_stream(const StepPlan& p, hipStream_t st, double* x, double* y, double* z, int32_t* cell, const int64_t* gid,
                              double* vel, int64_t n, double dt, double sigma, uint32_t step0, int nCyc, uint32_t seed,
                              const MeshView& m, unsigned long long* counters, const VertexField* vf, StreamState& ss, bool zSettled,
                              hipEvent_t evStart, hipEvent_t evStop) {
    return with_bools([&](auto B, auto R, auto SV, auto ST) {
        if (p.kernel == StepPlan::kStreamVertex)
            return with_lookup<0, 1>(p.lookup, [&](auto LF) {
                return launch_stream_inst<B, R, SV, ST, LF, true>(st, x, y, z, cell, gid, vel, n, dt, sigma, step0, nCyc, seed, m,
                                                                  counters, ss, vf, zSettled, evStart, evStop);
            });
        return with_lookup<0, 1, 2, 3, 4, 5, 6, 8, 9, 11>(p.lookup, [&](auto LF) {
            if constexpr (B && (LF == 8 || LF == 9)) return hipErrorInvalidValue;
            else return launch_stream_inst<B, R, SV, ST, LF>(st, x, y, z, cell, gid, vel, n, dt, sigma, step0, nCyc, seed, m, counters,
                                                             ss, vf, zSettled, evStart, evStop);
        });
    }, p.brown, p.reflect, p.storeVel, p.stats);
}

}
```

cudaparticlesfoam_amd/csrc/cpf_stream_ops.h:

```cpp
#pragma once
#include "cpf_walk.h"

namespace cpf {

#ifndef CPF_STREAM_GROUPS
#define CPF_STREAM_GROUPS 256
#endif
constexpr int kStreamGroups = CPF_STREAM_GROUPS;
constexpr int kStreamCounterStride = 16;

typedef __attribute__((address_space(3))) const char* lds_cptr;
__device__ __forceinline__ unsigned lds_addr(const void* p) {
    return (unsigned)(uintptr_t)(lds_cptr)p;
}
__device__ __forceinline__ unsigned uniform32(unsigned v) { return (unsigned)__builtin_amdgcn_readfirstlane((int)v); }
__device__ __forceinline__ int64_t uniform64(int64_t v) {
    const unsigned lo = uniform32((unsigned)v), hi = uniform32((unsigned)((uint64_t)v >> 32));
    return (int64_t)(((uint64_t)hi << 32) | lo);
}
__device__ __forceinline__ void glds16(const void* gsrc, unsigned ldsDst) {
    unsigned keep;
    asm volatile("s_waitcnt lgkmcnt(0)\n\ts_mov_b32 %0, m0\n\ts_mov_b32 m0, %2\n\ts_nop 0\n\t"
                 "global_load_lds_dwordx4 %1, off\n\ts_mov_b32 m0, %0"
                 : "=&s"(keep) : "v"(gsrc), "s"(ldsDst) : "memory");
}
__device__ __forceinline__ void async_store(double* base, unsigned byteOff, double v) {
    asm volatile("s_nop 4\n\tglobal_store_dwordx2 %0, %1, %2" : : "v"(byteOff), "v"(v), "s"(base) : "memory");
}
__device__ __forceinline__ void async_store(int32_t* base, unsigned byteOff, int v) {
    asm volatile("s_nop 4\n\tglobal_store_dword %0, %1, %2" : : "v"(byteOff), "v"(v), "s"(base) : "memory");
}
__device__ __forceinline__ unsigned grab_sync(unsigned* base) {
    unsigned r;
    asm volatile("s_nop 4\n\tglobal_atomic_add %0, %1, %2, %3 sc0\n\ts_waitcnt vmcnt(0)" : "=&v"(r) : "v"(0u), "v"(1u), "s"(base) : "memory");
    return r;
}
__device__ __forceinline__ void load3_sync(const double* base, unsigned byteOff, double& a, double& b, double& c) {
    asm volatile("s_waitcnt vmcnt(0)\n\ts_nop 4\n\tglobal_load_dwordx2 %0, %3, %4 sc0 sc1\n\tglobal_load_dwordx2 %1, %3, %4 offset:512 sc0 sc1\n\t"
                 "global_load_dwordx2 %2, %3, %4 offset:1024 sc0 sc1\n\ts_waitcnt vmcnt(0)"
                 : "=&v"(a), "=&v"(b), "=&v"(c) : "v"(byteOff), "s"(base) : "memory");
}
struct CloudPtrs { double* x; double* y; double* z; int32_t* cell; };
__device__ __forceinline__ CloudPtrs kernarg_cloud_ptrs() {
    typedef unsigned u32x8 __attribute__((ext_vector_type(8)));
    u32x8 r;
    asm volatile("s_load_dwordx8 %0, %1, 0x0\n\ts_waitcnt lgkmcnt(0)" : "=s"(r) : "s"(__builtin_amdgcn_kernarg_segment_ptr()) : "memory");
    auto ptr = [](unsigned lo, unsigned hi) { return (uintptr_t)(((unsigned long long)hi << 32) | lo); };
    return {reinterpret_cast<double*>(ptr(r[0], r[1])), reinterpret_cast<double*>(ptr(r[2], r[3])),
            reinterpret_cast<double*>(ptr(r[4], r[5])), reinterpret_cast<int32_t*>(ptr(r[6], r[7]))};
}
template <int BYTE_OFFSET>
__device__ __forceinline__ void* kernarg_pointer() {
    typedef unsigned u32x2 __attribute__((ext_vector_type(2)));
    u32x2 r;
    asm volatile("s_load_dwordx2 %0, %1, %2\n\ts_waitcnt lgkmcnt(0)" : "=s"(r) : "s"(__builtin_amdgcn_kernarg_segment_ptr()), "n"(BYTE_OFFSET) : "memory");
    return reinterpret_cast<void*>((uintptr_t)(((unsigned long long)r[1] << 32) | r[0]));
}
template <int OFF_A, int OFF_B>
__device__ __forceinline__ void kernarg_u32_pair(uint32_t& a, uint32_t& b) {
    asm volatile("s_load_dword %0, %2, %3\n\ts_load_dword %1, %2, %4\n\ts_waitcnt lgkmcnt(0)"
                 : "=&s"(a), "=&s"(b) : "s"(__builtin_amdgcn_kernarg_segment_ptr()), "n"(OFF_A), "n"(OFF_B) : "memory");
}
template <int BYTE_OFFSET>
__device__ __forceinline__ double kernarg_f64() {
    typedef unsigned u32x2 __attribute__((ext_vector_type(2)));
    u32x2 r;
    asm volatile("s_load_dwordx2 %0, %1, %2\n\ts_waitcnt lgkmcnt(0)" : "=s"(r) : "s"(__builtin_amdgcn_kernarg_segment_ptr()), "n"(BYTE_OFFSET) : "memory");
    return __longlong_as_double((long long)(((unsigned long long)r[1] << 32) | r[0]));
}
template <int N>
__device__ __forceinline__ void wait_vmcnt() { asm volatile("s_waitcnt vmcnt(%0)" : : "n"(N) : "memory"); }

struct StreamArgs {
    unsigned* grab;
    unsigned* grabNext;
    int wavesPerGroup;
    int tilesPerChunk;
    unsigned bigChunks;
    int debug;
    double* hitSpill;
    int zSettled;
};

inline hipError_t stream_launch_done(hipStream_t st, StreamState& ss) {
    const hipError_t e = hipGetLastError();
    if (e == hipSuccess) { ss.parity ^= 1; return e; }
    (void)hipMemsetAsync(ss.d_grab, 0, kStreamGrabBytes, st);
    return e;
}

}
```

Before: 96680.

## Add z-settled flat stream kernel specialization dropping z arithmetic and storage

```diff
diff --git a/cudaparticlesfoam_amd/csrc/cpf_api.cpp b/cudaparticlesfoam_amd/csrc/cpf_api.cpp
--- a/cudaparticlesfoam_amd/csrc/cpf_api.cpp
+++ b/cudaparticlesfoam_amd/csrc/cpf_api.cpp
@@ -74,6 +74,9 @@
     int lastStepCycles = 1;
     bool zSettled = false;
     bool lastStepZSettled = false;
+    unsigned* h_zBad = nullptr;
+    hipEvent_t evZBad = nullptr;
+    bool zBadPending = false;
     double* d_tetPos = nullptr; int32_t* d_tets = nullptr; double* d_vertVel = nullptr;
     int64_t nTetVerts = 0, nTets = 0; int tetsPerCell = 0; bool haveVertVel = false;
     double* d_vertCone = nullptr;
@@ -393,6 +396,13 @@
     ctx->streamState.flatField = ctx->h_occupied[2] == 0;
     ctx->fieldFlagPending = false;
 }
+bool zBadArrived(cpf_context* ctx) {
+    if (ctx->zBadPending) {
+        (void)hipEventSynchronize(ctx->evZBad);
+        ctx->zBadPending = false;
+    }
+    return *static_cast<volatile unsigned*>(ctx->h_zBad) != 0u;
+}
 void pollFieldFlag(cpf_context* ctx) {
     if (ctx->fieldFlagPending && hipEventQuery(ctx->evFieldFlag) == hipSuccess) fieldFlagArrived(ctx);
 }
@@ -423,6 +433,9 @@
     if (e == hipSuccess) e = hipHostMalloc((void**)&ctx->h_occupied, 32, hipHostMallocDefault);
     if (e == hipSuccess) { ctx->h_occupied[0] = ctx->h_occupied[1] = 0; ctx->h_occupied[2] = 1; ctx->streamState.occupiedHost = ctx->h_occupied; }
     if (e == hipSuccess) e = hipEventCreateWithFlags(&ctx->evFieldFlag, hipEventDisableTiming);
+    if (e == hipSuccess) e = hipHostMalloc((void**)&ctx->h_zBad, 64, hipHostMallocDefault);
+    if (e == hipSuccess) { *ctx->h_zBad = 0u; ctx->streamState.zBad = ctx->h_zBad; }
+    if (e == hipSuccess) e = hipEventCreateWithFlags(&ctx->evZBad, hipEventDisableTiming);
     if (e == hipSuccess) e = hipMalloc((void**)&ctx->streamState.d_grab, cpf::kStreamGrabBytes);
     if (e == hipSuccess) e = hipMemset(ctx->streamState.d_grab, 0, cpf::kStreamGrabBytes);
     if (e == hipSuccess) {
@@ -456,6 +469,8 @@
     freeDev(ctx->d_occupied);
     if (ctx->evFieldFlag) { (void)hipEventDestroy(ctx->evFieldFlag); ctx->evFieldFlag = nullptr; }
     if (ctx->h_occupied) { (void)hipHostFree(ctx->h_occupied); ctx->h_occupied = nullptr; ctx->streamState.occupiedHost = nullptr; }
+    if (ctx->evZBad) { (void)hipEventDestroy(ctx->evZBad); ctx->evZBad = nullptr; }
+    if (ctx->h_zBad) { (void)hipHostFree(ctx->h_zBad); ctx->h_zBad = nullptr; ctx->streamState.zBad = nullptr; }
     freeDev(ctx->d_tetPos); freeDev(ctx->d_tets); freeDev(ctx->d_vertVel); freeDev(ctx->d_vertCone); freeDev(ctx->d_vertApex);
     freeDev(ctx->snapDev);
     if (ctx->snapHost) { (void)hipHostFree(ctx->snapHost); ctx->snapHost = nullptr; }
@@ -823,6 +838,9 @@
     for (int c = 0; c < nLaunch; ++c) {
         const cpf::StepPlan plan = cpf::plan_step(m, ctx->streamState, ctx->stepVariant, vertexU ? &vf : nullptr, n, cycPerLaunch, D,
                                                   flags, ctx->stats);
+        if (plan.flat_body(ctx->streamState, settled) && zBadArrived(ctx)) settled = false;
+        const bool reportsZ = n > 0 && cycPerLaunch > 0 && plan.flat() && !settled && ctx->streamState.flatZ != 0;
+        if (reportsZ && !ctx->zBadPending) *static_cast<volatile unsigned*>(ctx->h_zBad) = 0u;
         hipEvent_t e0 = nullptr, e1 = nullptr;
         const bool timed = ctx->timing && (ctx->timingLaunch++ % (uint64_t)ctx->timingStride) == 0;
         const bool stamped = timed && n > 0 && plan.stamped();
@@ -844,6 +862,10 @@
         }
         CPF_HIP(ctx, le);
         if (n > 0 && cycPerLaunch > 0) settled = plan.flat();
+        if (reportsZ) {
+            CPF_HIP(ctx, hipEventRecord(ctx->evZBad, ctx->stream));
+            ctx->zBadPending = true;
+        }
         if (timed) {
             if (!stamped) CPF_HIP(ctx, hipEventRecord(e1, ctx->stream));
             ctx->events.emplace_back(e0, e1);
@@ -1159,6 +1181,8 @@
                  p.cone ? "cone locate" : (ctx->d_vertCone || ctx->vertConeWhy.empty() ? "all tets" : ("all tets: " + ctx->vertConeWhy).c_str()));
     else if (p.kernel == cpf::StepPlan::kAhead)
         snprintf(tmp, sizeof tmp, "cpf::step_kernel_ahead<%s, %s>", b[p.reflect], b[p.stats]);
+    else if (p.flat_body(ctx->streamState, ctx->zSettled) && !zBadArrived(ctx))
+        snprintf(tmp, sizeof tmp, "cpf::step_kernel_stream_flat<%s, %s, %s, %d>", b[p.reflect], b[p.storeVel], b[p.stats], p.lookup);
     else if (p.kernel == cpf::StepPlan::kStream)
         snprintf(tmp, sizeof tmp, "cpf::step_kernel_stream<%s, %s, %s, %s, %d>", b[p.brown], b[p.reflect], b[p.storeVel], b[p.stats], p.lookup);
     else if (p.kernel == cpf::StepPlan::kCoop)
diff --git a/cudaparticlesfoam_amd/csrc/cpf_device.h b/cudaparticlesfoam_amd/csrc/cpf_device.h
--- a/cudaparticlesfoam_amd/csrc/cpf_device.h
+++ b/cudaparticlesfoam_amd/csrc/cpf_device.h
@@ -55,6 +55,7 @@
     bool flatField = false;
     int flat = 1;
     int flatZ = 1;
+    unsigned* zBad = nullptr;
 };
 
 constexpr int kCoopMaxCells = 1 << 24;
@@ -69,6 +70,7 @@
     bool cone = false;
     bool stamped() const { return kernel == kStream || kernel == kStreamVertex; }
     bool flat() const { return kernel == kStream && (lookup == 8 || lookup == 9); }
+    bool flat_body(const StreamState& ss, bool zSettled) const { return flat() && zSettled && ss.flatZ != 0; }
 };
 StepPlan plan_step(const MeshView& m, const StreamState& ss, int variant, const VertexField* vf, int64_t n, int nCyc, double D,
                    unsigned flags, bool stats);
diff --git a/cudaparticlesfoam_amd/csrc/cpf_stream.hip b/cudaparticlesfoam_amd/csrc/cpf_stream.hip
--- a/cudaparticlesfoam_amd/csrc/cpf_stream.hip
+++ b/cudaparticlesfoam_amd/csrc/cpf_stream.hip
@@ -49,6 +49,7 @@
 };
 static_assert(offsetof(StreamKernArgs, x) == 0 && offsetof(StreamKernArgs, cell) == 24, "kernarg_cloud_ptrs reads bytes 0..31");
 constexpr int kKernArgHitSpill = (int)(offsetof(StreamKernArgs, sa) + offsetof(StreamArgs, hitSpill));
+constexpr int kKernArgZBad = (int)(offsetof(StreamKernArgs, sa) + offsetof(StreamArgs, zBad));
 constexpr int kKernArgGid = (int)offsetof(StreamKernArgs, gid), kKernArgSigma = (int)offsetof(StreamKernArgs, sigma);
 constexpr int kKernArgStep0 = (int)offsetof(StreamKernArgs, step0), kKernArgSeed = (int)offsetof(StreamKernArgs, seed);
 #ifndef CPF_STREAM_BROWN_KERNARG
@@ -99,6 +100,9 @@
 #endif
 #ifndef CPF_STREAM_WAVES_FLAT
 #define CPF_STREAM_WAVES_FLAT CPF_STREAM_WAVES
+#endif
+#ifndef CPF_STREAM_WAVES_FLAT_BODY
+#define CPF_STREAM_WAVES_FLAT_BODY 0
 #endif
 template <bool BROWNIAN, bool STORE_VEL, bool STATS, int LOOKUP>
 struct StreamOccupancy {
@@ -106,7 +110,7 @@
     static constexpr int waves = (STORE_VEL || STATS) ? 1 : (LOOKUP == 4 ? (BROWNIAN ? 4 : 5) : (BROWNIAN ? (kMixed ? 5 : ((LOOKUP == 6 || LOOKUP == 11) ? CPF_STREAM_WAVES_BOX_B : (LOOKUP == 1 ? CPF_STREAM_WAVES_B1 : CPF_STREAM_WAVES_B0))) : (LOOKUP == 2 ? CPF_STREAM_WAVES_L2 : ((kMixed && LOOKUP != 11) ? 6 : ((LOOKUP == 6 || LOOKUP == 11) ? CPF_STREAM_WAVES_BOX : (LOOKUP == 8 ? CPF_STREAM_WAVES_FLAT : CPF_STREAM_WAVES))))));
 };
 
-template <bool BROWNIAN, bool REFLECT, bool STORE_VEL, bool STATS, int LOOKUP, bool VERTEX>
+template <bool BROWNIAN, bool REFLECT, bool STORE_VEL, bool STATS, int LOOKUP, bool VERTEX, bool ZSET = false>
 __device__ __forceinline__ void stream_body(
     const int64_t* __restrict__ gid, double* __restrict__ vel, int64_t n, double dt, double sigma, uint32_t step0,
     int nCyc, uint32_t seed, const MeshView& m, unsigned long long* __restrict__ counters, const StreamArgs& sa, const VertexField& vf) {
@@ -127,10 +131,11 @@
     constexpr bool kInRound = CPF_STREAM_INROUND == 2 || (CPF_STREAM_INROUND == 1 && BROWNIAN);
     static_assert(!(kInRound && (LOOKUP == 2 || LOOKUP == 3 || LOOKUP == 5 || LOOKUP == 11)), "in-round reflection knows neither face groups nor two-record cells");
     constexpr int kPool = HIT_IN_REGS ? 1 : ((LOOKUP == 2 || LOOKUP == 3 || LOOKUP == 5 || LOOKUP == 11) ? 16 : ((BROWNIAN && LOOKUP == 0) ? CPF_STREAM_HIT_POOL_B0 : CPF_STREAM_HIT_POOL));
-    __shared__ double sLane[3][64];
+    static_assert(!ZSET || ((LOOKUP == 8 || LOOKUP == 9) && !BROWNIAN && !VERTEX), "settled z: the flat walk without the kick or the vertex advect");
+    __shared__ double sLane[ZSET ? 2 : 3][64];
     __shared__ double sPool[3][kPool];
     __shared__ unsigned sPoolUsed;
-    __shared__ double sPre[BROWNIAN ? 288 : 224];
+    __shared__ double sPre[ZSET ? 160 : (BROWNIAN ? 288 : 224)];
     __shared__ double sCone[VERTEX ? kVertexBlocks : 1][VERTEX ? kVertexTets * 10 : 1];
     double(*sE)[64] = sLane;
     const int lane = threadIdx.x;
@@ -140,7 +145,15 @@
     const int tpc = sa.tilesPerChunk;
     constexpr bool LOOKUP_FIXED = LOOKUP != 0 && LOOKUP != 5 && LOOKUP != 8;
     constexpr bool FLAT = LOOKUP == 8 || LOOKUP == 9;
-    const bool zKeep = FLAT && CPF_STREAM_FLAT_Z != 0 && sa.zSettled != 0;
+    const bool zKeep = ZSET || (FLAT && CPF_STREAM_FLAT_Z != 0 && sa.zSettled != 0);
+    auto park = [&](const D3& e) __attribute__((always_inline)) {
+        sE[0][lane] = e.x; sE[1][lane] = e.y;
+        if (!ZSET) sE[2][lane] = e.z;
+    };
+    auto parked = [&]() __attribute__((always_inline)) -> D3 {
+        if (ZSET) return {sE[0][lane], sE[1][lane], 0.0};
+        return {sE[0][lane], sE[1][lane], sE[2][lane]};
+    };
     constexpr bool mixed = LOOKUP == 2 || LOOKUP == 3 || LOOKUP == 5 || LOOKUP == 11;
     constexpr bool bigCells = LOOKUP == 2;
     constexpr int kGatherAhead = LOOKUP == 4 ? 3 : 0;
@@ -255,6 +268,10 @@
                 pid = haveIds ? (uint64_t) reinterpret_cast<const int64_t*>(sPre + 224)[ul] : (uint64_t)tile * 64 + ul;
             }
             if (ul > plim || pc < 0) pc = CPF_CELL_FROZEN;
+            if (FLAT && !ZSET && !zKeep && ballot64(pc >= 0 && !(fabs(pz) <= 1.7976931348623157e308)) != 0ull) {
+                unsigned* const bad = static_cast<unsigned*>(kernarg_pointer<kKernArgZBad>());
+                if (bad != nullptr && lane == 0) *bad = 1u;
+            }
 
             int cur = pc;
             int key2 = 0, carNext = 0, carBest = -1;
@@ -381,7 +398,7 @@
                 bool tlSat = false;
 #endif
                 const unsigned long long busyMask = ballot64(busy);
-                const D3 Epre = {sE[0][lane], sE[1][lane], sE[2][lane]};
+                const D3 Epre = parked();
                 const int lk = (bigCells && key2 != 0) ? key2 : cur;
                 int myslot = -1;
                 unsigned used = 0;
@@ -477,6 +494,12 @@
                 const uint64_t tlw0 = __builtin_amdgcn_s_memrealtime();
 #endif
                 if (nJobs != 0) {
+                    if (ZSET) {
+                        if (younger == 5) wait_vmcnt<5>();
+                        else if (younger == 3) wait_vmcnt<3>();
+                        else if (younger == 2) wait_vmcnt<2>();
+                        else wait_vmcnt<0>();
+                    } else
                     if (younger >= 7) wait_vmcnt<7>();
                     else if (younger == 6) wait_vmcnt<6>();
                     else if (younger == 5) wait_vmcnt<5>();
@@ -498,14 +521,15 @@
                         if (BOX) { const double2 uxy = reinterpret_cast<const double2*>(rec)[5]; u = {uxy.x, uxy.y, reinterpret_cast<const double*>(rec)[12], 0.0}; }
                         else u = rec[6];
                         v = {u.x, u.y, u.z};
-                        Pn = axpy(dt, v, S_);
-                    }
-                    D3 disp = {Pn.x - S_.x, Pn.y - S_.y, Pn.z - S_.z};
+                        if (ZSET) Pn = {fma(dt, v.x, S_.x), fma(dt, v.y, S_.y), 0.0};
+                        else Pn = axpy(dt, v, S_);
+                    }
+                    D3 disp = {Pn.x - S_.x, Pn.y - S_.y, ZSET ? 0.0 : Pn.z - S_.z};
                     if (BROWNIAN) {
                         const D3 xi = {sE[0][lane], sE[1][lane], sE[2][lane]};
                         disp = axpy(CPF_STREAM_BROWN_KERNARG ? kernarg_f64<kKernArgSigma>() : sigma, xi, disp);
                     }
-                    D3 E = {S_.x + disp.x, S_.y + disp.y, S_.z + disp.z};
+                    D3 E = {S_.x + disp.x, S_.y + disp.y, ZSET ? 0.0 : S_.z + disp.z};
                     if (BROWNIAN && REFLECT && zFold) {
                         bool clear;
                         const int nb = fold_z(E.z, rec[BOX ? 0 : 4], rec[BOX ? 0 : 5], clear);
@@ -513,7 +537,7 @@
                         if (STATS) st.refl += nb;
                         if (STORE_VEL && (nb & 1)) v.z = -v.z;
                     }
-                    sE[0][lane] = E.x; sE[1][lane] = E.y; sE[2][lane] = E.z;
+                    park(E);
                     return E;
                 };
                 if (busy) {
@@ -574,7 +598,7 @@
                                 } else if (BOX) wallPlane = box_wall_plane(rec, outSlot);
                                 else wallPlane = rec[outSlot];
                                 asm volatile("" ::: "memory");
-                                E = {sE[0][lane], sE[1][lane], sE[2][lane]};
+                                E = parked();
                                 if (kInRound) {
                                     park_hit(S_);
                                     if (STATS) ++st.refl;
@@ -631,9 +655,10 @@
                             park_hit(S_);
                             if (STATS) ++st.refl;
                             const D3 nn = {wallPlane.x, wallPlane.y, wallPlane.z};
-                            const double sd = dot3(wallPlane, E) - wallPlane.w;
-                            E = axpy(-2.0 * sd, nn, E);
-                            sE[0][lane] = E.x; sE[1][lane] = E.y; sE[2][lane] = E.z;
+                            const double sd = (ZSET ? fma(wallPlane.y, E.y, wallPlane.x * E.x) : dot3(wallPlane, E)) - wallPlane.w;
+                            if (ZSET) E = {fma(-2.0 * sd, nn.x, E.x), fma(-2.0 * sd, nn.y, E.y), 0.0};
+                            else E = axpy(-2.0 * sd, nn, E);
+                            park(E);
                             v = axpy(-2.0 * dot3(wallPlane, v), nn, v);
                             h = 0;
                             ++j;
@@ -659,14 +684,14 @@
 
             auto cycle_end = [&]() __attribute__((always_inline)) {
                 if (cur >= 0) {
-                    const D3 E = {sE[0][lane], sE[1][lane], sE[2][lane]};
+                    const D3 E = parked();
                     if (REFLECT && j != 0) {
                         D3 hit;
                         if (HIT_IN_REGS) hit = hitReg;
                         else if (hitAt < kPool) hit = {sPool[0][hitAt], sPool[1][hitAt], sPool[2][hitAt]};
                         else load3_sync(static_cast<const double*>(kernarg_pointer<kKernArgHitSpill>()) + (size_t)blockIdx.x * kStreamHitSpillDoubles,
                                         ul * 8u, hit.x, hit.y, hit.z);
-                        S_ = {hit.x + (E.x - hit.x), hit.y + (E.y - hit.y), hit.z + (E.z - hit.z)};
+                        S_ = {hit.x + (E.x - hit.x), hit.y + (E.y - hit.y), ZSET ? 0.0 : hit.z + (E.z - hit.z)};
                     } else S_ = E;
                     if (j >= kMaxReflect) { cur = CPF_CELL_LOST; if (STATS) ++st.lost; }
                 }
@@ -703,7 +728,7 @@
 #endif
                 }
             } else {
-                const D3 prev = {sE[0][lane], sE[1][lane], sE[2][lane]};
+                const D3 prev = parked();
                 (void)hook(prev);
             }
 
@@ -716,7 +741,7 @@
             ++tlTiles;
 #endif
             rtile = tile; havePrev = true;
-            sE[0][lane] = S_.x; sE[1][lane] = S_.y; sE[2][lane] = S_.z;
+            park(S_);
             if (STORE_VEL) { rvx = v.x; rvy = v.y; rvz = v.z; ralive = pc >= 0; }
             rc = cur;
             rlim = plim;
@@ -727,10 +752,10 @@
             const int64_t b = (int64_t)rtile * 64;
             const CloudPtrs cp = kernarg_cloud_ptrs();
             double* const x = cp.x; double* const y = cp.y; double* const z = cp.z; int32_t* const cell = cp.cell;
-            const double rx = sE[0][lane], ry = sE[1][lane], rz = sE[2][lane];
+            const D3 res = parked();
             if (ul <= rlim) {
-                (x + b)[ul] = rx; (y + b)[ul] = ry;
-                if (!zKeep) (z + b)[ul] = rz;
+                (x + b)[ul] = res.x; (y + b)[ul] = res.y;
+                if (!zKeep) (z + b)[ul] = res.z;
                 (cell + b)[ul] = rc;
             }
             if (STORE_VEL && ralive) {
@@ -768,7 +793,15 @@
     stream_body<BROWNIAN, REFLECT, STORE_VEL, STATS, LOOKUP, true>(gid, vel, n, dt, sigma, step0, nCyc, seed, m, counters, sa, vf);
 }
 
-template <bool B, bool R_, bool SV, bool ST, int LF, bool VX = false>
+template <bool REFLECT, bool STORE_VEL, bool STATS, int LOOKUP>
+__global__ __launch_bounds__(64, (StreamOccupancy<false, STORE_VEL, STATS, LOOKUP>::waves)) void step_kernel_stream_flat(
+    double* __restrict__ , double* __restrict__ , double* __restrict__ , int32_t* __restrict__ ,
+    const int64_t* __restrict__ gid, double* __restrict__ vel, int64_t n, double dt, double sigma, uint32_t step0,
+    int nCyc, uint32_t seed, MeshView m, unsigned long long* __restrict__ counters, StreamArgs sa) {
+    stream_body<false, REFLECT, STORE_VEL, STATS, LOOKUP, false, true>(gid, vel, n, dt, sigma, step0, nCyc, seed, m, counters, sa, VertexField{});
+}
+
+template <bool B, bool R_, bool SV, bool ST, int LF, bool VX = false, bool ZS = false>
 static hipError_t launch_stream_inst(hipStream_t st, double* x, double* y, double* z, int32_t* cell, const int64_t* gid,
                                      double* vel, int64_t n, double dt, double sigma, uint32_t step0, int nCyc,
                                      uint32_t seed, const MeshView& m, unsigned long long* counters, StreamState& ss,
@@ -778,9 +811,11 @@
         int nb = 0;
         hipError_t e;
         if constexpr (VX) e = hipOccupancyMaxActiveBlocksPerMultiprocessor(&nb, step_kernel_stream_vertex<B, R_, SV, ST, LF>, 64, 0);
+        else if constexpr (ZS) e = hipOccupancyMaxActiveBlocksPerMultiprocessor(&nb, step_kernel_stream_flat<R_, SV, ST, LF>, 64, 0);
         else e = hipOccupancyMaxActiveBlocksPerMultiprocessor(&nb, step_kernel_stream<B, R_, SV, ST, LF>, 64, 0);
         if (e != hipSuccess) return e;
         wavesPerCU = nb < 1 ? 1 : (nb > 32 ? 32 : nb);
+        if (ZS && CPF_STREAM_WAVES_FLAT_BODY > 0 && wavesPerCU > 4 * CPF_STREAM_WAVES_FLAT_BODY) wavesPerCU = 4 * CPF_STREAM_WAVES_FLAT_BODY;
     }
     const int64_t nTiles = (n + 63) >> 6;
     if (nTiles >= ((int64_t)1 << 31)) return hipErrorInvalidValue;
@@ -800,7 +835,8 @@
     if (R * kStreamGroups > ss.hitSpillWaves) R = ss.hitSpillWaves / kStreamGroups;
     if (R < 1 || ss.d_hitSpill == nullptr) return hipErrorInvalidValue;
     const bool zSettled = (LF == 8 || LF == 9) && !VX && settled && ss.flatZ != 0;
-    StreamArgs sa = {cur, nxt, (int)R, tpc, (unsigned)bigChunks, ss.debug, ss.d_hitSpill, zSettled ? 1 : 0};
+    if (ZS != zSettled && (LF == 8 || LF == 9) && !VX) return hipErrorInvalidValue;
+    StreamArgs sa = {cur, nxt, (int)R, tpc, (unsigned)bigChunks, ss.debug, ss.d_hitSpill, zSettled ? 1 : 0, ss.zBad};
     if constexpr (VX) {
         if (vf == nullptr) return hipErrorInvalidValue;
         if (evStart != nullptr && evStop != nullptr)
@@ -809,6 +845,14 @@
         else
         hipLaunchKernelGGL((step_kernel_stream_vertex<B, R_, SV, ST, LF>), dim3((unsigned)(R * kStreamGroups)), dim3(64), 0, st, x, y, z, cell,
                            gid, vel, n, dt, sigma, step0, nCyc, seed, m, counters, sa, *vf);
+        return stream_launch_done(st, ss);
+    } else if constexpr (ZS) {
+        if (evStart != nullptr && evStop != nullptr)
+            hipExtLaunchKernelGGL((step_kernel_stream_flat<R_, SV, ST, LF>), dim3((unsigned)(R * kStreamGroups)), dim3(64), 0, st, evStart,
+                                  evStop, 0, x, y, z, cell, gid, vel, n, dt, sigma, step0, nCyc, seed, m, counters, sa);
+        else
+        hipLaunchKernelGGL((step_kernel_stream_flat<R_, SV, ST, LF>), dim3((unsigned)(R * kStreamGroups)), dim3(64), 0, st, x, y, z, cell,
+                           gid, vel, n, dt, sigma, step0, nCyc, seed, m, counters, sa);
         return stream_launch_done(st, ss);
     } else {
     if (evStart != nullptr && evStop != nullptr)
@@ -888,6 +932,12 @@
                 return launch_stream_inst<B, R, SV, ST, LF, true>(st, x, y, z, cell, gid, vel, n, dt, sigma, step0, nCyc, seed, m,
                                                                   counters, ss, vf, zSettled, evStart, evStop);
             });
+        if (p.flat_body(ss, zSettled))
+            return with_lookup<8, 9>(p.lookup, [&](auto LF) {
+                if constexpr (B) return hipErrorInvalidValue;
+                else return launch_stream_inst<false, R, SV, ST, LF, false, true>(st, x, y, z, cell, gid, vel, n, dt, sigma, step0, nCyc, seed, m,
+                                                                                  counters, ss, vf, zSettled, evStart, evStop);
+            });
         return with_lookup<0, 1, 2, 3, 4, 5, 6, 8, 9, 11>(p.lookup, [&](auto LF) {
             if constexpr (B && (LF == 8 || LF == 9)) return hipErrorInvalidValue;
             else return launch_stream_inst<B, R, SV, ST, LF>(st, x, y, z, cell, gid, vel, n, dt, sigma, step0, nCyc, seed, m, counters,
diff --git a/cudaparticlesfoam_amd/csrc/cpf_stream_ops.h b/cudaparticlesfoam_amd/csrc/cpf_stream_ops.h
--- a/cudaparticlesfoam_amd/csrc/cpf_stream_ops.h
+++ b/cudaparticlesfoam_amd/csrc/cpf_stream_ops.h
@@ -80,6 +80,7 @@
     int debug;
     double* hitSpill;
     int zSettled;
+    unsigned* zBad;
 };
 
 inline hipError_t stream_launch_done(hipStream_t st, StreamState& ss) {
```

New measurement: 105,400, median of 6. +9.1%, better.
